# bytewax/bytewax

Hardware: AMD Instinct MI355X
Metric: events/sec (whole node), tumbling-window wordcount (higher is better)
Workload: dtype int64; 1 GPU; model=tumbling-window wordcount (keyed count, 60s windows), events_per_batch_per_gpu=64000000, vocab=1000000, parallelism=key-hash all-to-allv dp1, engine=dataflow (run_main: source -> keyed_window_agg -> sink), radix=True, radix_v2=False, latency_method=poll-gap under load, closed_window_rows=317000000

## Files before the change

### bytewax_amd/_native/stream_kernels.hip

```cpp

#include <hip/hip_runtime.h>
#include <torch/extension.h>
#include <pybind11/stl.h>
#include <ATen/hip/HIPContext.h>

#include <chrono>
#include <type_traits>
#include <cstdlib>
#include <cstdint>
#include <cstring>
#include <vector>

#define WAVE 64
#define EMPTY_SLOT 0xFFFFFFFFFFFFFFFFULL

#define HIP_CHECK(expr)                                               \
  do {                                                                \
    hipError_t _e = (expr);                                           \
    TORCH_CHECK(_e == hipSuccess, "HIP error: ", hipGetErrorString(_e)); \
  } while (0)

static inline int n_blocks(int64_t n, int block) {
  int64_t b = (n + block - 1) / block;
  if (b > 2048) b = 2048;
// ... 349 lines not shown
      int rp = atomicAdd(&gres[b], 1);
      if (rp < res_cap) {
        ev_res[(int64_t)b * res_cap + rp] = stage[b][q];
      } else {
        atomicOr(error_flag, 1);
      }
    }
  }
  for (int off = WAVE / 2; off > 0; off >>= 1) {
    int64_t other = __shfl_down((long long)local_max, off);
    if (other > local_max) local_max = other;
  }
  if ((threadIdx.x & (WAVE - 1)) == 0 && local_max > 0) {
    atomicMax(max_ts, (unsigned long long)local_max);
  }
}

#define V2_CACHE 4096

__global__ __launch_bounds__(256) void k_agg_cached(
    const uint64_t* __restrict__ ev,
    const uint64_t* __restrict__ ev_res,
    const int* __restrict__ gcur,
    const int* __restrict__ gres,
    int64_t cap_c,
    int64_t res_cap,
    int slices,
    uint64_t* __restrict__ tkeys,
    unsigned long long* __restrict__ tvals,
    uint64_t mask,
    int region_bits,
    int* __restrict__ error_flag) {
  __shared__ uint64_t ckeys[V2_CACHE];
  __shared__ unsigned long long cvals[V2_CACHE];
  for (int s = threadIdx.x; s < V2_CACHE; s += blockDim.x) {
    ckeys[s] = EMPTY_SLOT;
    cvals[s] = 0;
  }
  __syncthreads();
  int cb = blockIdx.x % V2_COARSE;
  int slice = blockIdx.x / V2_COARSE;

  auto agg_one = [&](uint64_t packed) {
    uint64_t h64 = mix64(packed);
    int lh = (int)((h64 >> 20) & (V2_CACHE - 1));
    for (int p = 0; p < 2; ++p) {
      uint64_t cur = ckeys[lh];
      if (cur == packed) {
        atomicAdd(&cvals[lh], 1ULL);
        return;
      }
      if (cur == EMPTY_SLOT) {
        uint64_t prev = atomicCAS(
            (unsigned long long*)&ckeys[lh], EMPTY_SLOT, packed);
        if (prev == EMPTY_SLOT || prev == packed) {
          atomicAdd(&cvals[lh], 1ULL);
          return;
        }
      }
      lh = (lh + 1) & (V2_CACHE - 1);
    }
    if (!hash_add(tkeys, tvals, mask, region_bits, packed, 1ULL)) {
      atomicOr(error_flag, 1);
    }
  };

  int c = gcur[cb];
  if (c > cap_c) c = (int)cap_c;
  for (int j = slice * (int)blockDim.x + threadIdx.x; j < c;
       j += slices * (int)blockDim.x) {
    agg_one(ev[(int64_t)cb * cap_c + j]);
  }
  int cr = gres[cb];
  if (cr > res_cap) cr = (int)res_cap;
  for (int j = slice * (int)blockDim.x + threadIdx.x; j < cr;
       j += slices * (int)blockDim.x) {
    agg_one(ev_res[(int64_t)cb * res_cap + j]);
  }
  __syncthreads();
  for (int s = threadIdx.x; s < V2_CACHE; s += blockDim.x) {
    if (ckeys[s] != EMPTY_SLOT) {
      if (!hash_add(tkeys, tvals, mask, region_bits, ckeys[s], cvals[s])) {
        atomicOr(error_flag, 1);
      }
    }
  }
}

__device__ __forceinline__ int64_t win_lo_of(
    int64_t t, int64_t align_ms, int64_t len_ms, int64_t off_ms) {
  int64_t num = t - align_ms - len_ms;
  int64_t fl = num >= 0 ? num / off_ms : -((-num + off_ms - 1) / off_ms);
  return fl + 1;
}

__device__ __forceinline__ int64_t win_of(
    int64_t t, int64_t align_ms, int64_t len_ms, uint64_t m2,
    uint64_t maxfast) {
  int64_t x = t - align_ms;
  if (m2 != 0 && (uint64_t)x < maxfast) {
    return (int64_t)__umul64hi((uint64_t)x, m2);
  }
  return x / len_ms;
}

static inline void magic_div_u64(
    int64_t d, uint64_t* m2, uint64_t* maxfast) {
  *m2 = 0;
  *maxfast = 0;
  if (d <= 1) return;
  if ((d & (d - 1)) == 0) {
    int s = 0;
    while ((int64_t(1) << s) < d) ++s;
    *m2 = (uint64_t)1 << (64 - s);
    *maxfast = ~(uint64_t)0;
    return;
  }
  const unsigned p = 60;
  unsigned __int128 one = 1;
  uint64_t M = (uint64_t)(((one << p) + (uint64_t)d - 1) / (uint64_t)d);
  uint64_t e = (uint64_t)((unsigned __int128)M * (uint64_t)d - (one << p));
  *m2 = M << 4;
  *maxfast = e ? (uint64_t)((one << p) / e) : ~(uint64_t)0;
}

struct Win32 {
  uint32_t dlo;
  uint32_t dspan;
  uint32_t c;
  uint32_t wlo;
  uint32_t qoff;
  uint32_t dm;
  int sh1, sh2;
};

__device__ __forceinline__ uint32_t win32_div(uint32_t y, const Win32& w) {
  uint32_t t = __umulhi(w.dm, y);
  return (t + ((y - t) >> w.sh1)) >> w.sh2;
}

#define ENTRY_SLOT_BITS 13
#define ENTRY_SLOT_MASK 0x1FFFull
#define ENTRY_DELTA_MASK 0x7FFFFu
#define ENTRY_DELTA_LIMIT 0x7FFFFu
#define ENTRY_W_CLASSIC INT64_MIN

__device__ __forceinline__ uint32_t entry_delta(uint64_t entry) {
  return ((uint32_t)entry >> ENTRY_SLOT_BITS) & ENTRY_DELTA_MASK;
}

__device__ __forceinline__ uint64_t entry_classic(
    uint64_t entry, uint32_t wlo) {
  return ((uint64_t)(wlo + entry_delta(entry)) << 32) | (entry >> 32);
}

template <int MODE, typename TS = int64_t, bool LATE = false>
__global__ void k_radix_scatter_fixed(
    const int32_t* __restrict__ keys,
    const TS* __restrict__ ts,
    const int64_t* __restrict__ vals,
    int64_t n,
    int64_t align_ms,
    int64_t len_ms,
    int64_t off_ms,
    int64_t ts_base,
    uint64_t mask,
    int region_bits,
    int64_t cap,
    int* __restrict__ gcursors,
    uint64_t* __restrict__ ev_packed,
    int64_t* __restrict__ ev_vals,
    int* __restrict__ ov_cursor,
    uint64_t* __restrict__ ov_packed,
    int64_t* __restrict__ ov_vals,
    int64_t ov_cap,
    unsigned long long* __restrict__ max_ts,
    int* __restrict__ error_flag,
    uint64_t win_m2,
    uint64_t win_maxfast,
    int64_t late_cutoff,
    int32_t* __restrict__ late_keys,
    int64_t* __restrict__ late_ts,
    int64_t* __restrict__ late_vals,
    int* __restrict__ late_n,
    int64_t late_cap) {
  static_assert(!(LATE && MODE == AGG_TS), "no late tracking for AGG_TS");
  extern __shared__ int lmem[];
  __shared__ int s_late[LATE ? 2 : 1];
  int nb = (int)(((mask + 1) >> region_bits));
  int* lhist = lmem;
  int* lbase = lmem + nb;
  for (int b = threadIdx.x; b < nb; b += blockDim.x) lhist[b] = 0;
  if constexpr (LATE) {
    if (threadIdx.x == 0) s_late[0] = 0;
  }
  __syncthreads();
  int64_t start = blockIdx.x * (int64_t)blockDim.x + threadIdx.x;
  int64_t stride = gridDim.x * (int64_t)blockDim.x;
  int64_t local_max = 0;
  for (int64_t i = start; i < n; i += stride) {
    int64_t t = (int64_t)ts[i] + ts_base;
    if constexpr (LATE) {
      bool is_late = t < late_cutoff;
      wave_reserve(is_late, &s_late[0]);
      if (is_late) continue;
    }
    if (t > local_max) local_max = t;
    uint64_t packed;
    int nwin = 1;
    if (MODE == AGG_TS) {
      packed = (uint64_t)(uint32_t)keys[i];
    } else {
      int64_t win = win_of(t, align_ms, off_ms, win_m2, win_maxfast);
      packed = ((uint64_t)(uint32_t)(int32_t)win << 32) | (uint32_t)keys[i];
      if (off_ms < len_ms) {
        nwin = (int)(win - win_lo_of(t, align_ms, len_ms, off_ms)) + 1;
      }
    }
    for (int w = 0; w < nwin; ++w) {
      atomicAdd(&lhist[(int)region_of(mix64(packed), mask, region_bits)], 1);
      packed -= (uint64_t)1 << 32;
    }
  }
  __syncthreads();
  for (int b = threadIdx.x; b < nb; b += blockDim.x) {
    lbase[b] = lhist[b] > 0 ? atomicAdd(&gcursors[b], lhist[b]) : 0;
    lhist[b] = 0;
  }
  if constexpr (LATE) {
    if (threadIdx.x == 0) {
      s_late[1] = s_late[0] > 0 ? atomicAdd(late_n, s_late[0]) : 0;
      s_late[0] = 0;
    }
  }
  __syncthreads();
  for (int64_t i = start; i < n; i += stride) {
    int64_t t = (int64_t)ts[i] + ts_base;
    if constexpr (LATE) {
      bool is_late = t < late_cutoff;
      int lpos = wave_reserve(is_late, &s_late[0]);
      if (is_late) {
        late_store<MODE == AGG_SUM>(
            (int64_t)s_late[1] + lpos, keys[i], t,
            MODE == AGG_SUM ? vals[i] : 0, late_keys, late_ts, late_vals,
            late_cap, error_flag);
        continue;
      }
    }
    uint64_t packed;
    int nwin = 1;
    if (MODE == AGG_TS) {
      packed = (uint64_t)(uint32_t)keys[i];
    } else {
      int64_t win = win_of(t, align_ms, off_ms, win_m2, win_maxfast);
      packed = ((uint64_t)(uint32_t)(int32_t)win << 32) | (uint32_t)keys[i];
      if (off_ms < len_ms) {
        nwin = (int)(win - win_lo_of(t, align_ms, len_ms, off_ms)) + 1;
      }
    }
    int64_t v = (MODE == AGG_SUM) ? vals[i] : (MODE == AGG_TS ? t : 0);
    for (int w = 0; w < nwin; ++w) {
      int b = (int)region_of(mix64(packed), mask, region_bits);
      int64_t in_bucket = lbase[b] + atomicAdd(&lhist[b], 1);
      if (in_bucket < cap) {
        int64_t pos = (int64_t)b * cap + in_bucket;
        ev_packed[pos] = packed;
        if (MODE != AGG_COUNT) ev_vals[pos] = v;
      } else {
        int opos = atomicAdd(ov_cursor, 1);
        if (opos < ov_cap) {
          ov_packed[opos] = packed;
          if (MODE != AGG_COUNT) ov_vals[opos] = v;
        } else {
          atomicOr(error_flag, 1);
        }
      }
      packed -= (uint64_t)1 << 32;
    }
  }
  for (int off = WAVE / 2; off > 0; off >>= 1) {
    int64_t other = __shfl_down((long long)local_max, off);
    if (other > local_max) local_max = other;
  }
  if ((threadIdx.x & (WAVE - 1)) == 0 && local_max > 0) {
    atomicMax(max_ts, (unsigned long long)local_max);
  }
}

template <int MODE, typename TS = int64_t>
__global__ void k_radix_scatter_direct(
    const int32_t* __restrict__ keys,
    const TS* __restrict__ ts,
    const int64_t* __restrict__ vals,
    int64_t n,
    int64_t align_ms,
    int64_t len_ms,
    int64_t off_ms,
    int64_t ts_base,
    uint64_t mask,
    int region_bits,
    int64_t cap,
    int* __restrict__ gcursors,
    uint64_t* __restrict__ ev_packed,
    int64_t* __restrict__ ev_vals,
    int* __restrict__ ov_cursor,
    uint64_t* __restrict__ ov_packed,
// ... 324 lines not shown
      int64_t i = t0 + u * BLK + tid;
      if (i > n - 1) i = n - 1;
      rk[u] = keys[i];
      rt[u] = ts[i];
    }
  };
  const int64_t stride = (int64_t)gridDim.x * T;
  int64_t local_max = 0;
  int64_t t0 = (int64_t)blockIdx.x * T;
  const bool seen = t0 + tid < n;
  if (t0 < n) {
    load_tile(t0);
    if (HASHED) local_max = (int64_t)rt[0];
  }
  for (; t0 < n; t0 += stride) {
    uint64_t pk[U];
    int sr[U];
    if (!HASHED) {
#pragma unroll
      for (int u = 0; u < U; ++u) {
        int64_t i = t0 + u * BLK + tid;
        int64_t t = (int64_t)rt[u] + ts_base;
        int64_t win = win_of(t, align_ms, len_ms, win_m2, win_maxfast);
        uint64_t packed =
            ((uint64_t)(uint32_t)(int32_t)win << 32) | (uint32_t)rk[u];
        pk[u] = packed;
        int b = (int)region_of(mix64(packed), mask, seg_bits);
        sr[u] = -1;
        if (i < n) {
          if (t > local_max) local_max = t;
          sr[u] = (atomicAdd(&lhist[b], 1) << 13) | b;
        }
      }
    } else {
      int64_t left64 = n - t0 - tid;
      const int left = left64 > T ? T : (left64 < 0 ? 0 : (int)left64);
      int32_t dmax = (int32_t)local_max;
      uint32_t rare = 0;
#pragma unroll
      for (int u = 0; u < U; ++u) {
        const bool in = u * BLK < left;
        const uint32_t d = (uint32_t)rt[u];
        const uint32_t q = win32_div(d + w32.c, w32);
        const uint64_t packed =
            ((uint64_t)(w32.wlo + q) << 32) | (uint32_t)rk[u];
        const uint64_t h64 = mix64(packed);
        const uint32_t delta = q - w32.qoff;
        const bool fits =
            d - w32.dlo < w32.dspan && delta < ENTRY_DELTA_LIMIT;
        pk[u] = ((uint64_t)(uint32_t)rk[u] << 32) |
                (uint64_t)(delta << ENTRY_SLOT_BITS) |
                ((h64 >> 32) & ENTRY_SLOT_MASK);
        if (in && !fits) rare |= 1u << u;
        if (in && (int32_t)d > dmax) dmax = (int32_t)d;
        const bool ok = in && fits;
        int b = (int)region_of(h64, mask, seg_bits);
        int rank = atomicAdd(&lhist[b], ok ? 1 : 0);
        sr[u] = ok ? ((rank << 13) | b) : -1;
      }
      local_max = dmax;
      while (rare != 0) {
        int u = __ffs(rare) - 1;
        rare &= rare - 1;
        int64_t i = t0 + u * BLK + tid;
        int64_t win = win_of((int64_t)ts[i] + ts_base, align_ms, len_ms,
                             win_m2, win_maxfast);
        spill(((uint64_t)(uint32_t)(int32_t)win << 32) | (uint32_t)keys[i]);
      }
    }
    if (t0 + stride < n) load_tile(t0 + stride);
    __syncthreads();
    int rc = 0, grant = 0, gb = 0;
    if (tid < nseg) {
      rc = res_cnt[tid];
      int tot = rc + lhist[tid];
      grant = tot & ~(SC_GRAN - 1);
      if (grant > 0) gb = atomicAdd(&gcursors[tid], grant);
      res_cnt[tid] = tot - grant;
      lhist[tid] = 0;
    }
    int incl = grant;
    for (int o = 1; o < WAVE; o <<= 1) {
      int v = __shfl_up(incl, o);
      if (lane >= o) incl += v;
    }
    if (lane == WAVE - 1) s_wtot[wave] = incl;
    __syncthreads();
    int total = 0, woff = 0;
    for (int w = 0; w < NW; ++w) {
      int v = s_wtot[w];
      if (w < wave) woff += v;
      total += v;
    }
    if (tid < nseg) {
      int off = woff + incl - grant;
      lpack[tid] = off | (rc << 14) | (grant << 17);
      if (grant > 0) {
#pragma unroll
        for (int j = 0; j < SC_GRAN - 1; ++j)
          stage[off + j] = res[(size_t)tid * SC_GRAN + j];
        for (int j = 0; j < grant; j += SC_GRAN) {
          int64_t gp = (int64_t)gb + j;
          gdst[(off + j) / SC_GRAN] =
              gp < cap ? (uint32_t)(((int64_t)tid * cap + gp) / SC_GRAN)
                       : GD_SPILL;
        }
      }
    }
    __syncthreads();
    for (int u = 0; u < U; ++u) {
      if (sr[u] < 0) continue;
      int b = sr[u] & ((1 << 13) - 1);
      int w = lpack[b];
      int vpos = ((w >> 14) & 7) + (sr[u] >> 13);
      int g = w >> 17;
      if (vpos < g) stage[(w & ((1 << 14) - 1)) + vpos] = pk[u];
      else res[(size_t)b * SC_GRAN + (vpos - g)] = pk[u];
    }
    __syncthreads();
    for (int p = tid; p < total / 2; p += BLK) {
      ulonglong2 v = *(const ulonglong2*)(stage + 2 * p);
      uint32_t d = gdst[p / 4];
      if (d != GD_SPILL) {
        *(ulonglong2*)(ev_packed + (int64_t)d * SC_GRAN + 2 * (p & 3)) = v;
      } else {
        if (v.x != EMPTY_SLOT) spill(classic_of(v.x));
        if (v.y != EMPTY_SLOT) spill(classic_of(v.y));
      }
    }
  }
  __syncthreads();
  if (tid < nseg) {
    int rc = res_cnt[tid];
    if (rc > 0) {
      int gb = atomicAdd(&gcursors[tid], SC_GRAN);
      for (int j = 0; j < SC_GRAN; ++j) {
        uint64_t p = j < rc ? res[(size_t)tid * SC_GRAN + j] : EMPTY_SLOT;
        int64_t gp = (int64_t)gb + j;
        if (gp < cap) ev_packed[(int64_t)tid * cap + gp] = p;
        else if (p != EMPTY_SLOT) spill(classic_of(p));
      }
    }
  }
  if (HASHED) local_max = seen ? local_max + ts_base : 0;
  for (int off = WAVE / 2; off > 0; off >>= 1) {
    int64_t other = __shfl_down((long long)local_max, off);
    if (other > local_max) local_max = other;
  }
  if ((threadIdx.x & (WAVE - 1)) == 0 && local_max > 0) {
    atomicMax(max_ts, (unsigned long long)local_max);
  }
}

template <int MODE>
__global__ void k_overflow_agg(
    const uint64_t* __restrict__ ov_packed,
    const int64_t* __restrict__ ov_vals,
    const int* __restrict__ ov_cursor,
    int64_t ov_cap,
    uint64_t* __restrict__ tkeys,
    unsigned long long* __restrict__ tvals,
    uint64_t mask,
    int region_bits,
    int* __restrict__ error_flag) {
  int64_t n = *ov_cursor;
  if (n > ov_cap) n = ov_cap;
  int64_t i = blockIdx.x * (int64_t)blockDim.x + threadIdx.x;
  int64_t stride = gridDim.x * (int64_t)blockDim.x;
  for (; i < n; i += stride) {
    unsigned long long inc =
        (MODE == AGG_SUM) ? (unsigned long long)ov_vals[i] : 1ULL;
    if (!hash_add(tkeys, tvals, mask, region_bits, ov_packed[i], inc)) {
      atomicOr(error_flag, 1);
    }
  }
}

typedef unsigned long long agg_u64x2 __attribute__((ext_vector_type(2)));

template <int MODE>
__global__ __launch_bounds__(1024) void k_radix_agg(
    const uint64_t* __restrict__ ev_packed,
    const int64_t* __restrict__ ev_vals,
    const int* __restrict__ counts,
    int64_t cap,
    uint64_t* __restrict__ tkeys,
    unsigned long long* __restrict__ tvals,
    uint64_t mask,
    int region_bits,
    int lds_bits,
    int* __restrict__ error_flag) {
  extern __shared__ char smem[];
  int region = 1 << lds_bits;
  uint64_t* lkeys = (uint64_t*)smem;
  unsigned long long* lvals =
      (unsigned long long*)(smem + (size_t)region * sizeof(uint64_t));
  for (int s = threadIdx.x; s < region; s += blockDim.x) {
    lkeys[s] = EMPTY_SLOT;
    lvals[s] = 0;
  }
  __syncthreads();
  int b = blockIdx.x;
  int cnt = counts[b];
  if (cnt > (int)cap) cnt = (int)cap;
  const uint64_t* seg = ev_packed + (int64_t)b * cap;
  const int64_t* segv =
      (MODE == AGG_SUM) ? ev_vals + (int64_t)b * cap : nullptr;

  auto add = [&](uint64_t packed, unsigned long long inc) {
    if (packed == EMPTY_SLOT) return;
    uint64_t h64 = mix64(packed);
    int lh = (int)((h64 >> 32) & (region - 1));
    bool done = false;
    for (int p = 0; p < region; ++p) {
      uint64_t cur = lkeys[lh];
      if (cur == packed) {
        atomicAdd(&lvals[lh], inc);
        done = true;
        break;
      }
      if (cur == EMPTY_SLOT) {
        uint64_t prev = atomicCAS(
            (unsigned long long*)&lkeys[lh], EMPTY_SLOT, packed);
        if (prev == EMPTY_SLOT || prev == packed) {
          atomicAdd(&lvals[lh], inc);
          done = true;
          break;
        }
      }
      lh = (lh + 1) & (region - 1);
    }
    if (!done) {
      if (!hash_add(tkeys, tvals, mask, region_bits, packed, inc)) {
        atomicOr(error_flag, 1);
      }
    }
  };

  const int head = (cnt > 0 && ((uintptr_t)seg & 15) != 0) ? 1 : 0;
  const int nvec = (cnt - head) >> 1;
  const int tail = head + 2 * nvec;
  if (threadIdx.x == 0 && head) {
    add(seg[0], MODE == AGG_SUM ? (unsigned long long)segv[0] : 1ULL);
  }
  if (threadIdx.x == blockDim.x - 1 && tail < cnt) {
    add(seg[tail],
        MODE == AGG_SUM ? (unsigned long long)segv[tail] : 1ULL);
  }

  constexpr int R = (MODE == AGG_SUM) ? 2 : 4;
  const agg_u64x2* vseg = (const agg_u64x2*)(seg + head);
  const int64_t* vval = (MODE == AGG_SUM) ? segv + head : nullptr;
  const int T = (int)blockDim.x;
  const int chunk = R * T;
  agg_u64x2 cur_p[R], nxt_p[R];
  unsigned long long cur_v[R][2], nxt_v[R][2];
  auto fetch = [&](agg_u64x2 (&bp)[R], unsigned long long (&bv)[R][2],
                   int base) {
#pragma unroll
    for (int r = 0; r < R; ++r) {
      int v = base + r * T + (int)threadIdx.x;
      if (v < nvec) {
        bp[r] = vseg[v];
        if (MODE == AGG_SUM) {
          bv[r][0] = (unsigned long long)vval[2 * v];
          bv[r][1] = (unsigned long long)vval[2 * v + 1];
        }
      } else {
        bp[r] = agg_u64x2{EMPTY_SLOT, EMPTY_SLOT};
        if (MODE == AGG_SUM) bv[r][0] = bv[r][1] = 0;
      }
    }
  };
  if (nvec > 0) fetch(cur_p, cur_v, 0);
  for (int base = 0; base < nvec; base += chunk) {
    if (base + chunk < nvec) fetch(nxt_p, nxt_v, base + chunk);
#pragma unroll
    for (int r = 0; r < R; ++r) {
      add(cur_p[r].x, MODE == AGG_SUM ? cur_v[r][0] : 1ULL);
      add(cur_p[r].y, MODE == AGG_SUM ? cur_v[r][1] : 1ULL);
    }
#pragma unroll
    for (int r = 0; r < R; ++r) {
      cur_p[r] = nxt_p[r];
      if (MODE == AGG_SUM) {
        cur_v[r][0] = nxt_v[r][0];
        cur_v[r][1] = nxt_v[r][1];
      }
    }
  }
  __syncthreads();
  for (int s = threadIdx.x; s < region; s += blockDim.x) {
    if (lkeys[s] != EMPTY_SLOT) {
      if (!hash_add(tkeys, tvals, mask, region_bits, lkeys[s], lvals[s])) {
        atomicOr(error_flag, 1);
      }
    }
  }
}

#define AGG_DELTA_MAX 14u
#define AGG_DELTA_MID 7u

template <int BLK, int R, bool HASHED = false>
__global__ __launch_bounds__(BLK, BLK == 1024 ? 8 : 4) void k_radix_agg_count(
    const uint64_t* __restrict__ ev_packed,
    const int* __restrict__ counts,
    int64_t cap,
    uint64_t* __restrict__ tkeys,
    unsigned long long* __restrict__ tvals,
    uint64_t mask,
    int region_bits,
    int lds_bits,
    int* __restrict__ error_flag,
    uint32_t wlo) {
  extern __shared__ char smem[];
  unsigned long long* cells = (unsigned long long*)smem;
  const int region = 1 << lds_bits;
  const uint32_t lmask = (uint32_t)region - 1;
  const int b = blockIdx.x;
  int cnt = counts[b];
  if (cnt > (int)cap) cnt = (int)cap;
  if (cnt <= 0) return;
  for (int s = threadIdx.x; s < region / 2; s += BLK) {
    ((agg_u64x2*)cells)[s] = agg_u64x2{EMPTY_SLOT, EMPTY_SLOT};
  }
  const uint64_t* seg = ev_packed + (int64_t)b * cap;
  auto win_part = [&](uint64_t packed) {
    return HASHED ? entry_delta(packed) : (uint32_t)(packed >> 32);
  };
  auto key_part = [&](uint64_t packed) {
    return HASHED ? (uint32_t)(packed >> 32) : (uint32_t)packed;
  };
  const uint32_t wbase = win_part(seg[0]) - AGG_DELTA_MID;
  __syncthreads();

  auto escape = [&](uint64_t packed) {
    if (HASHED) packed = entry_classic(packed, wlo);
    if (!hash_add(tkeys, tvals, mask, region_bits, packed, 1ULL)) {
      atomicOr(error_flag, 1);
    }
  };
  auto slot_of = [&](uint64_t packed) {
    if (HASHED) return (uint32_t)packed & lmask;
    return (uint32_t)(mix64(packed) >> 32) & lmask;
  };
  auto tag_of = [&](uint64_t packed) {
    return ((unsigned long long)key_part(packed) << 4) |
           (unsigned long long)(win_part(packed) - wbase);
  };
  auto drain = [&](uint32_t pend, auto entry, auto start, auto skipped) {
    uint64_t packed = 0;
    unsigned long long tag = 0;
    uint32_t lh = 0;
    int left = 0;
    while (left != 0 || pend != 0) {
      if (left == 0) {
        int e = __ffs(pend) - 1;
        pend &= pend - 1;
        packed = entry(e);
        if (win_part(packed) - wbase > AGG_DELTA_MAX) {
          escape(packed);
          continue;
        }
        tag = tag_of(packed);
        lh = start(e);
        left = region - (skipped(e) ? 1 : 0);
      }
      unsigned long long cur = cells[lh];
      if (cur == EMPTY_SLOT) {
        cur = atomicCAS(&cells[lh], EMPTY_SLOT, tag << 28);
        if (cur == EMPTY_SLOT) cur = tag << 28;
      }
      if ((cur >> 28) == tag) {
        atomicAdd((unsigned int*)&cells[lh], 1u);
        left = 0;
      } else {
        lh = (lh + 1) & lmask;
        if (--left == 0) escape(packed);
      }
    }
  };
  auto add_one = [&](uint64_t packed) {
    if (packed == EMPTY_SLOT) return;
    drain(
        1u, [&](int) { return packed; },
        [&](int) { return slot_of(packed); }, [&](int) { return false; });
  };

  const int head = ((uintptr_t)seg & 15) != 0 ? 1 : 0;
  const int nvec = (cnt - head) >> 1;
  const int tail = head + 2 * nvec;
  if (threadIdx.x == 0 && head) add_one(seg[0]);
  if (threadIdx.x == BLK - 1 && tail < cnt) add_one(seg[tail]);

  const agg_u64x2* vseg = (const agg_u64x2*)(seg + head);
  constexpr int chunk = R * BLK;
  constexpr int E = 2 * R;
  agg_u64x2 cur_p[R], nxt_p[R];
  auto fetch = [&](agg_u64x2 (&bp)[R], int base) {
#pragma unroll
    for (int r = 0; r < R; ++r) {
      int v = base + r * BLK + (int)threadIdx.x;
      if (v < nvec) bp[r] = vseg[v];
      else bp[r] = agg_u64x2{EMPTY_SLOT, EMPTY_SLOT};
    }
  };
  fetch(cur_p, 0);
  for (int base = 0; base < nvec; base += chunk) {
    if (base + chunk < nvec) fetch(nxt_p, base + chunk);
    uint32_t slot[E];
    unsigned long long first[E];
#pragma unroll
    for (int e = 0; e < E; ++e) {
      uint64_t packed = (e & 1) ? cur_p[e >> 1].y : cur_p[e >> 1].x;
      slot[e] = slot_of(packed);
      first[e] = cells[slot[e]];
    }
    uint32_t pend = 0, moved = 0;
#pragma unroll
    for (int e = 0; e < E; ++e) {
      uint64_t packed = (e & 1) ? cur_p[e >> 1].y : cur_p[e >> 1].x;
      if (packed == EMPTY_SLOT) continue;
      bool in_range = win_part(packed) - wbase <= AGG_DELTA_MAX;
      if (in_range && (first[e] >> 28) == tag_of(packed)) {
        atomicAdd((unsigned int*)&cells[slot[e]], 1u);
      } else {
        pend |= 1u << e;
        if (first[e] != EMPTY_SLOT) {
          slot[e] = (slot[e] + 1) & lmask;
          moved |= 1u << e;
        }
      }
    }
    if (pend != 0) {
      drain(
          pend,
          [&](int e) {
            uint64_t v = 0;
#pragma unroll
            for (int j = 0; j < E; ++j) {
              if (j == e) v = (j & 1) ? cur_p[j >> 1].y : cur_p[j >> 1].x;
            }
            return v;
          },
          [&](int e) {
            uint32_t v = 0;
#pragma unroll
            for (int j = 0; j < E; ++j) {
              if (j == e) v = slot[j];
            }
            return v;
          },
          [&](int e) { return ((moved >> e) & 1u) != 0; });
    }
#pragma unroll
    for (int r = 0; r < R; ++r) cur_p[r] = nxt_p[r];
  }
  __syncthreads();

  for (int s = threadIdx.x; s < region; s += BLK) {
    unsigned long long c = cells[s];
    if (c != EMPTY_SLOT) {
      uint32_t win = wbase + ((uint32_t)c >> 28) + (HASHED ? wlo : 0u);
      uint64_t packed = ((uint64_t)win << 32) | (c >> 32);
      if (!hash_add(tkeys, tvals, mask, region_bits, packed,
                    c & 0x0FFFFFFFULL)) {
        atomicOr(error_flag, 1);
      }
    }
  }
}

__global__ void k_overflow_agg_stats(
    const uint64_t* __restrict__ ov_packed,
    const int64_t* __restrict__ ov_vals,
    const int* __restrict__ ov_cursor,
    int64_t ov_cap,
    uint64_t* __restrict__ tkeys,
    long long* __restrict__ tcnt,
    long long* __restrict__ tsum,
    long long* __restrict__ tmin,
    long long* __restrict__ tmax,
    uint64_t mask,
    int* __restrict__ error_flag) {
  int64_t n = *ov_cursor;
  if (n > ov_cap) n = ov_cap;
  int64_t i = blockIdx.x * (int64_t)blockDim.x + threadIdx.x;
  int64_t stride = gridDim.x * (int64_t)blockDim.x;
  for (; i < n; i += stride) {
    uint64_t slot = find_slot(tkeys, mask, ov_packed[i]);
    if (slot == ~0ULL) {
      atomicOr(error_flag, 1);
      continue;
    }
    long long v = ov_vals[i];
    atomicAdd((unsigned long long*)&tcnt[slot], 1ULL);
    atomicAdd((unsigned long long*)&tsum[slot], (unsigned long long)v);
    atomicMin(&tmin[slot], v);
    atomicMax(&tmax[slot], v);
  }
}

__global__ __launch_bounds__(1024) void k_radix_agg_stats(
    const uint64_t* __restrict__ ev_packed,
    const int64_t* __restrict__ ev_vals,
    const int* __restrict__ offsets,
    const int* __restrict__ counts,
    uint64_t* __restrict__ tkeys,
    long long* __restrict__ tcnt,
    long long* __restrict__ tsum,
    long long* __restrict__ tmin,
    long long* __restrict__ tmax,
    int64_t clamp_cap,
    uint64_t mask,
    int region_bits,
    int lds_bits,
    int* __restrict__ error_flag) {
  extern __shared__ char smem[];
  int region = 1 << lds_bits;
  uint64_t* lkeys = (uint64_t*)smem;
  long long* lcnt = (long long*)(smem + (size_t)region * 8);
  long long* lsum = (long long*)(smem + (size_t)region * 16);
  long long* lmin = (long long*)(smem + (size_t)region * 24);
  long long* lmax = (long long*)(smem + (size_t)region * 32);
  const long long LLMAX = 0x7FFFFFFFFFFFFFFFLL;
  for (int s = threadIdx.x; s < region; s += blockDim.x) {
    lkeys[s] = EMPTY_SLOT;
    lcnt[s] = 0;
    lsum[s] = 0;
    lmin[s] = LLMAX;
    lmax[s] = -LLMAX - 1;
  }
  __syncthreads();
  int b = blockIdx.x;
  int cnt = counts[b];
  if (clamp_cap > 0 && cnt > (int)clamp_cap) cnt = (int)clamp_cap;
  int start = offsets[b];
  for (int j = threadIdx.x; j < cnt; j += blockDim.x) {
    uint64_t packed = ev_packed[start + j];
    if (packed == EMPTY_SLOT) continue;
    long long v = ev_vals[start + j];
    uint64_t h64 = mix64(packed);
    int lh = (int)((h64 >> 32) & (region - 1));
    int slot = -1;
    for (int p = 0; p < region; ++p) {
      uint64_t cur = lkeys[lh];
      if (cur == packed) {
        slot = lh;
        break;
      }
      if (cur == EMPTY_SLOT) {
        uint64_t prev = atomicCAS(
            (unsigned long long*)&lkeys[lh], EMPTY_SLOT, packed);
        if (prev == EMPTY_SLOT || prev == packed) {
          slot = lh;
          break;
        }
      }
      lh = (lh + 1) & (region - 1);
    }
    if (slot >= 0) {
      atomicAdd((unsigned long long*)&lcnt[slot], 1ULL);
      atomicAdd((unsigned long long*)&lsum[slot], (unsigned long long)v);
      atomicMin(&lmin[slot], v);
      atomicMax(&lmax[slot], v);
    } else {
      uint64_t gslot = find_slot(tkeys, mask, packed);
      if (gslot == ~0ULL) {
        atomicOr(error_flag, 1);
      } else {
        atomicAdd((unsigned long long*)&tcnt[gslot], 1ULL);
        atomicAdd((unsigned long long*)&tsum[gslot], (unsigned long long)v);
        atomicMin(&tmin[gslot], v);
        atomicMax(&tmax[gslot], v);
      }
    }
  }
  __syncthreads();
  for (int s = threadIdx.x; s < region; s += blockDim.x) {
    if (lkeys[s] != EMPTY_SLOT) {
      uint64_t gslot = find_slot(tkeys, mask, lkeys[s]);
      if (gslot == ~0ULL) {
        atomicOr(error_flag, 1);
        continue;
      }
      atomicAdd((unsigned long long*)&tcnt[gslot],
                (unsigned long long)lcnt[s]);
      atomicAdd((unsigned long long*)&tsum[gslot],
                (unsigned long long)lsum[s]);
      atomicMin(&tmin[gslot], lmin[s]);
      atomicMax(&tmax[gslot], lmax[s]);
    }
  }
}

__global__ void k_close_extract(
    const uint64_t* __restrict__ tkeys,
    const unsigned long long* __restrict__ tvals,
    int64_t nslots,
    int64_t win_lo,
    int64_t win_hi,
    int32_t* __restrict__ out_keys,
    int32_t* __restrict__ out_wins,
    int64_t* __restrict__ out_vals,
    int* __restrict__ out_n,
    int64_t cap) {
  int64_t i = blockIdx.x * (int64_t)blockDim.x + threadIdx.x;
  int64_t stride = gridDim.x * (int64_t)blockDim.x;
  for (; i < nslots; i += stride) {
    uint64_t k = tkeys[i];
    bool take = false;
    int32_t win = 0;
    if (k != EMPTY_SLOT) {
      win = (int32_t)(uint32_t)(k >> 32);
      take = (int64_t)win >= win_lo && (int64_t)win < win_hi;
    }
    unsigned long long ball = __ballot(take);
    int lane = threadIdx.x & (WAVE - 1);
    if (ball != 0) {
// ... 1433 lines not shown
  return LateSink{late_cutoff, late_keys.data_ptr<int32_t>(),
                  late_ts.data_ptr<int64_t>(), vp,
                  late_n.data_ptr<int32_t>(), cap};
}

static void window_agg_insert_impl(
    torch::Tensor keys,
    torch::Tensor ts,
    c10::optional<torch::Tensor> vals,
    torch::Tensor tkeys,
    torch::Tensor tvals,
    torch::Tensor max_ts,
    torch::Tensor error_flag,
    int64_t align_ms,
    int64_t len_ms,
    int64_t mode,
    bool dedup,
    int64_t ts_base,
    int64_t region_bits,
    int64_t off_ms,
    const LateSink* late) {
  TORCH_CHECK(late == nullptr || !dedup,
              "late tracking is incompatible with the dedup path");
  if (off_ms <= 0) off_ms = len_ms;
  TORCH_CHECK(off_ms <= len_ms, "window offset must be <= length");
  TORCH_CHECK(off_ms == len_ms || !dedup,
              "sliding windows are incompatible with the dedup path");
  check_dev(keys, torch::kInt32, "keys");
  bool ts32 = ts.scalar_type() == torch::kInt32;
  if (!ts32) check_dev(ts, torch::kInt64, "ts");
  check_dev(tkeys, torch::kInt64, "tkeys");
  check_dev(tvals, torch::kInt64, "tvals");
  check_dev(max_ts, torch::kInt64, "max_ts");
  check_dev(error_flag, torch::kInt32, "error_flag");
  int64_t n = keys.numel();
  TORCH_CHECK(ts.numel() == n, "ts/keys length mismatch");
  int64_t nslots = tkeys.numel();
  TORCH_CHECK((nslots & (nslots - 1)) == 0, "table size must be 2^k");
  TORCH_CHECK(len_ms > 0, "window length must be positive");
  const int64_t* vptr = nullptr;
  if (mode == AGG_SUM) {
    TORCH_CHECK(vals.has_value(), "sum mode requires vals");
    check_dev(*vals, torch::kInt64, "vals");
    TORCH_CHECK(vals->numel() == n, "vals/keys length mismatch");
    vptr = vals->data_ptr<int64_t>();
  }
  if (n == 0) return;
  auto stream = at::hip::getCurrentHIPStream();
  dim3 block(256);
  dim3 grid(n_blocks(n, 256));
  auto launch = [&](auto kern, auto tsptr) {
    hipLaunchKernelGGL(
        kern, grid, block, 0, stream,
        keys.data_ptr<int32_t>(), tsptr, vptr, n,
        (uint64_t*)tkeys.data_ptr<int64_t>(),
        (unsigned long long*)tvals.data_ptr<int64_t>(),
        (uint64_t)(nslots - 1), align_ms, len_ms, off_ms, ts_base,
        (int)region_bits,
        (unsigned long long*)max_ts.data_ptr<int64_t>(),
        error_flag.data_ptr<int32_t>(), (const int64_t*)nullptr,
        late ? late->cutoff : (int64_t)0, late ? late->keys : nullptr,
        late ? late->ts : nullptr, late ? late->vals : nullptr,
        late ? late->n : nullptr, late ? late->cap : (int64_t)0);
  };
  auto dispatch = [&](auto tsptr) {
    using TSV = std::remove_const_t<std::remove_pointer_t<decltype(tsptr)>>;
    if (late != nullptr && mode == AGG_COUNT)
      launch((k_window_agg_insert<AGG_COUNT, false, TSV, true>), tsptr);
    else if (late != nullptr)
      launch((k_window_agg_insert<AGG_SUM, false, TSV, true>), tsptr);
    else if (mode == AGG_COUNT && !dedup)
      launch(k_window_agg_insert<AGG_COUNT, false, TSV>, tsptr);
    else if (mode == AGG_COUNT && dedup)
      launch(k_window_agg_insert<AGG_COUNT, true, TSV>, tsptr);
    else if (mode == AGG_SUM && !dedup)
      launch(k_window_agg_insert<AGG_SUM, false, TSV>, tsptr);
    else
      launch(k_window_agg_insert<AGG_SUM, true, TSV>, tsptr);
  };
  if (ts32) dispatch(ts.data_ptr<int32_t>());
  else dispatch(ts.data_ptr<int64_t>());
}

void window_agg_insert(
    torch::Tensor keys,
    torch::Tensor ts,
    c10::optional<torch::Tensor> vals,
    torch::Tensor tkeys,
    torch::Tensor tvals,
    torch::Tensor max_ts,
    torch::Tensor error_flag,
    int64_t align_ms,
    int64_t len_ms,
    int64_t mode,
    bool dedup,
    int64_t ts_base,
    int64_t region_bits,
    int64_t off_ms) {
  window_agg_insert_impl(keys, ts, vals, tkeys, tvals, max_ts, error_flag,
                         align_ms, len_ms, mode, dedup, ts_base, region_bits,
                         off_ms, nullptr);
}

void window_agg_insert_late(
    torch::Tensor keys,
    torch::Tensor ts,
    c10::optional<torch::Tensor> vals,
    torch::Tensor tkeys,
    torch::Tensor tvals,
    torch::Tensor max_ts,
    torch::Tensor error_flag,
    int64_t align_ms,
    int64_t len_ms,
    int64_t mode,
    int64_t ts_base,
    int64_t region_bits,
    int64_t off_ms,
    int64_t late_cutoff,
    torch::Tensor late_keys,
    torch::Tensor late_ts,
    c10::optional<torch::Tensor> late_vals,
    torch::Tensor late_n) {
  LateSink sink = make_late_sink(late_cutoff, late_keys, late_ts, late_vals,
                                 late_n, mode == AGG_SUM);
  window_agg_insert_impl(keys, ts, vals, tkeys, tvals, max_ts, error_flag,
                         align_ms, len_ms, mode, false, ts_base, region_bits,
                         off_ms, &sink);
}

static unsigned device_cu_count() {
  static int cus = 0;
  if (cus == 0) {
    int dev = 0, v = 0;
    if (hipGetDevice(&dev) == hipSuccess &&
        hipDeviceGetAttribute(&v, hipDeviceAttributeMultiprocessorCount,
                              dev) == hipSuccess &&
        v > 0)
      cus = v;
    else
      cus = 256;
  }
  return (unsigned)cus;
}

static bool agg_wide_env() {
  const char* s = std::getenv("BYTEWAX_AGG");
  return s != nullptr && s[0] == 'w';
}

static bool entries_classic_env() {
  const char* s = std::getenv("BYTEWAX_ENTRIES");
  return s != nullptr && s[0] == 'c';
}

static bool staged2_shape(int64_t nseg, int* threads, int* u, size_t* lds) {
  int env_u = 0, env_threads = 0;
  if (const char* e = std::getenv("BYTEWAX_SCATTER_U")) env_u = atoi(e);
  if (const char* e = std::getenv("BYTEWAX_SCATTER_THREADS"))
    env_threads = atoi(e);
  *threads = env_threads == 1024 ? 1024 : 512;
  *u = *threads == 512 && env_u != 8 ? 16 : 8;
  *lds = staged2_lds_bytes(nseg, (int64_t)*threads * *u);
  return nseg <= *threads && *lds <= 160 * 1024;
}

static bool count_staged2_ok(int64_t xf, const void* evp, int64_t nseg) {
  int threads, u;
  size_t lds;
  return xf == 1 && scatter_staged2_env() && (((uintptr_t)evp) & 15) == 0 &&
         staged2_shape(nseg, &threads, &u, &lds);
}

static bool count_agg_compact(int64_t cap, int seg_bits) {
  return !agg_wide_env() && cap < ((int64_t)1 << 28) && seg_bits >= 8 &&
         seg_bits <= 13;
}

struct CountEntries {
  bool hashed = false;
  int64_t W = 0;
  uint32_t qoff = 0;
  uint32_t dm = 0;
  int sh1 = 0, sh2 = 0;
  int64_t agg_w() const {
    return hashed ? W + (int64_t)qoff : ENTRY_W_CLASSIC;
  }
};

static CountEntries plan_count_entries(
    bool staged_count, int64_t xf, const void* evp, int64_t nseg,
    int64_t cap, int seg_bits, bool ts_i32, int64_t align_ms,
    int64_t len_ms, int64_t first_base) {
  CountEntries ce;
  if (!staged_count || !ts_i32 || entries_classic_env() ||
      !count_staged2_ok(xf, evp, nseg) || !count_agg_compact(cap, seg_bits))
    return ce;
  if (len_ms < 1 || len_ms >= ((int64_t)1 << 31)) return ce;
  int threads, u;
  size_t lds;
  staged2_shape(nseg, &threads, &u, &lds);
  if (threads != 512 || u != 16) return ce;
  __int128 num = (__int128)first_base - align_ms - ((__int128)1 << 31);
  __int128 w = num / len_ms;
  if (num % len_ms < 0) w -= 1;
  if (w < -((__int128)1 << 62) || w > ((__int128)1 << 62)) return ce;
  ce.hashed = true;
  ce.W = (int64_t)w;
  int l = 0;
  while (((int64_t)1 << l) < len_ms) ++l;
  ce.dm = (uint32_t)((((unsigned __int128)1 << 32) *
                      (uint64_t)(((int64_t)1 << l) - len_ms)) /
                     (uint64_t)len_ms) + 1u;
  ce.sh1 = l < 1 ? l : 1;
  ce.sh2 = l > 1 ? l - 1 : 0;
  int64_t q0 = (int64_t)((num - w * len_ms + ((__int128)1 << 31)) / len_ms);
  ce.qoff = q0 > (1 << 18) ? (uint32_t)(q0 - (1 << 18)) : 0u;
  return ce;
}

static Win32 make_win32(
    const CountEntries& ce, int64_t ts_base, int64_t align_ms,
    int64_t len_ms) {
  Win32 w{};
  __int128 c = (__int128)ts_base - align_ms - (__int128)ce.W * len_ms;
  __int128 lo = -((__int128)1 << 31), hi = ((__int128)1 << 31) - 1;
  if (-c > lo) lo = -c;
  if ((__int128)align_ms - ts_base > lo) lo = (__int128)align_ms - ts_base;
  __int128 top = ((__int128)1 << 32) - 1 - c;
  if (top < hi) hi = top;
  if (hi >= lo) {
    __int128 span = hi - lo + 1;
    if (span > 0xFFFFFFFFll) span = 0xFFFFFFFFll;
    w.dlo = (uint32_t)(int32_t)(int64_t)lo;
    w.dspan = (uint32_t)(uint64_t)span;
  }
  w.c = (uint32_t)(uint64_t)(c & 0xFFFFFFFFll);
  w.wlo = (uint32_t)(uint64_t)ce.W;
  w.qoff = ce.qoff;
  w.dm = ce.dm;
  w.sh1 = ce.sh1;
  w.sh2 = ce.sh2;
  return w;
}

template <typename TSV>
static void launch_count_staged(
    hipStream_t stream, const int32_t* keys, const TSV* ts, int64_t n,
    int64_t xf, int64_t align_ms, int64_t len_ms, int64_t off_ms,
    int64_t ts_base, uint64_t mask, int seg_bits, int64_t nseg, int64_t cap,
    int* gcur, uint64_t* evp, int* ovc, uint64_t* ovp, int64_t ov_cap,
    unsigned long long* max_ts, int* err, uint64_t win_m2,
    uint64_t win_maxfast, bool overlapped, const CountEntries& ce) {
  int env_u = 0, env_threads = 0, env_blocks = 0;
  if (const char* e = std::getenv("BYTEWAX_SCATTER_U")) env_u = atoi(e);
  if (const char* e = std::getenv("BYTEWAX_SCATTER_THREADS"))
    env_threads = atoi(e);
  if (const char* e = std::getenv("BYTEWAX_SCATTER_BLOCKS")) {
    int v = atoi(e);
    if (v > 0) env_blocks = v;
  }
  auto go = [&](auto kern, int threads, int u, unsigned cap_gs, size_t lds,
                auto... extra) {
    int64_t tile = (int64_t)threads * u;
    int64_t gs = (n * xf + tile - 1) / tile;
    if (env_blocks > 0) cap_gs = (unsigned)env_blocks;
    if (gs > (int64_t)cap_gs) gs = cap_gs;
    if (gs < 1) gs = 1;
    hipLaunchKernelGGL(
        kern, dim3((unsigned)gs), dim3((unsigned)threads), lds, stream, keys,
        ts, (const int64_t*)nullptr, n, align_ms, len_ms, off_ms, ts_base,
        mask, seg_bits, cap, gcur, evp, (int64_t*)nullptr, ovc, ovp,
        (int64_t*)nullptr, ov_cap, max_ts, err, win_m2, win_maxfast,
        extra...);
    HIP_CHECK(hipGetLastError());
  };
  TORCH_CHECK(!ce.hashed || count_staged2_ok(xf, evp, nseg),
              "hashed entries planned for a scatter that is not staged2");
  if (count_staged2_ok(xf, evp, nseg)) {
    const unsigned cus = device_cu_count() * (overlapped ? 2u : 1u);
    int threads, u;
    size_t lds;
    staged2_shape(nseg, &threads, &u, &lds);
    Win32 w32{};
    if constexpr (sizeof(TSV) == 4) {
      if (ce.hashed) {
        w32 = make_win32(ce, ts_base, align_ms, len_ms);
        go((k_radix_scatter_staged2<TSV, 16, 512, true>), 512, 16, cus, lds,
           w32);
        return;
      }
    }
    TORCH_CHECK(!ce.hashed, "hashed entries need int32 timestamp deltas");
    if (threads == 1024)
      go((k_radix_scatter_staged2<TSV, 8, 1024>), 1024, 8, cus, lds, w32);
    else if (u == 16)
      go((k_radix_scatter_staged2<TSV, 16, 512>), 512, 16, cus, lds, w32);
    else
      go((k_radix_scatter_staged2<TSV, 8, 512>), 512, 8, cus, lds, w32);
    return;
  }
  size_t lds = (size_t)nseg * SC_GRAN * 8 + 4 * (size_t)nseg * sizeof(int);
  int threads = 512;
  if (env_threads == 256 || env_threads == 1024) threads = env_threads;
  if (threads == 512)
    go((k_radix_scatter_staged<AGG_COUNT, TSV, 16, 512>), 512, 16, 1024u,
       lds, NO_LATE_ARGS);
  else if (threads == 1024)
    go((k_radix_scatter_staged<AGG_COUNT, TSV, 16, 1024>), 1024, 16, 1024u,
       lds, NO_LATE_ARGS);
  else if (env_u == 8)
    go((k_radix_scatter_staged<AGG_COUNT, TSV, 8>), 256, 8, 1024u, lds,
       NO_LATE_ARGS);
  else if (env_u == 32)
    go((k_radix_scatter_staged<AGG_COUNT, TSV, 32>), 256, 32, 1024u, lds,
       NO_LATE_ARGS);
  else
    go((k_radix_scatter_staged<AGG_COUNT, TSV, 16>), 256, 16, 1024u, lds,
       NO_LATE_ARGS);
}

static void launch_count_agg(
    hipStream_t stream, const uint64_t* evp, const int* gcur, int64_t cap,
    uint64_t* tkeys, unsigned long long* tvals, uint64_t mask,
    int region_bits, int seg_bits, int64_t nseg, int* err,
    int64_t entry_w) {
  const bool hashed = entry_w != ENTRY_W_CLASSIC;
  const uint32_t wlo = hashed ? (uint32_t)(uint64_t)entry_w : 0u;
  if (count_agg_compact(cap, seg_bits)) {
    auto go = [&](auto kern, int threads) {
      hipLaunchKernelGGL(
          kern, dim3((unsigned)nseg), dim3((unsigned)threads),
          (size_t)8 << seg_bits, stream, evp, gcur, cap, tkeys, tvals, mask,
          region_bits, seg_bits, err, wlo);
      HIP_CHECK(hipGetLastError());
    };
    if (seg_bits >= 12) {
      if (hashed) go((k_radix_agg_count<1024, 2, true>), 1024);
      else go((k_radix_agg_count<1024, 2>), 1024);
    } else {
      if (hashed) go((k_radix_agg_count<256, 2, true>), 256);
      else go((k_radix_agg_count<256, 2>), 256);
    }
    return;
  }
  TORCH_CHECK(!hashed, "hashed scatter entries need the compact aggregation");
  hipLaunchKernelGGL(
      k_radix_agg<AGG_COUNT>, dim3((unsigned)nseg),
      dim3(seg_bits >= 12 ? 1024u : 256u), (size_t)16 << seg_bits, stream,
      evp, (const int64_t*)nullptr, gcur, cap, tkeys, tvals, mask,
      region_bits, seg_bits, err);
  HIP_CHECK(hipGetLastError());
}

static dim3 overflow_agg_grid() { return dim3(device_cu_count()); }

static void radix_window_insert_impl(
    torch::Tensor keys,
    torch::Tensor ts,
    c10::optional<torch::Tensor> vals,
    torch::Tensor tkeys,
    torch::Tensor tvals,
    torch::Tensor max_ts,
    torch::Tensor error_flag,
    torch::Tensor gcursors,
    torch::Tensor ev_packed,
    torch::Tensor ev_vals,
    torch::Tensor ov_cursor,
    torch::Tensor ov_packed,
    torch::Tensor ov_vals,
    int64_t align_ms,
    int64_t len_ms,
    int64_t mode,
    int64_t ts_base,
    int64_t region_bits,
    int64_t off_ms,
    std::vector<int64_t> seg_counts,
    std::vector<int64_t> seg_bases,
    const LateSink* late) {
  if (off_ms <= 0) off_ms = len_ms;
  TORCH_CHECK(off_ms <= len_ms, "window offset must be <= length");
  check_dev(keys, torch::kInt32, "keys");
  bool seg32 = !seg_counts.empty();
  bool ts32 = ts.scalar_type() == torch::kInt32;
  if (seg32) {
    TORCH_CHECK(seg_counts.size() == seg_bases.size(),
                "seg_counts/seg_bases length mismatch");
    check_dev(ts, torch::kInt32, "ts32");
  } else if (!ts32) {
    check_dev(ts, torch::kInt64, "ts");
  }
  int64_t n = keys.numel();
  int64_t nslots = tkeys.numel();
  TORCH_CHECK((nslots & (nslots - 1)) == 0, "table size must be 2^k");
  TORCH_CHECK(region_bits > 0, "radix path requires region_bits > 0");
  TORCH_CHECK(region_bits <= 12, "region_bits > 12 exceeds the LDS "
              "budget of the aggregation kernel (16 B/slot)");
  int64_t nb = nslots >> region_bits;
  TORCH_CHECK(nb >= 1 && nb <= 8192, "region count out of range");
  TORCH_CHECK(gcursors.numel() >= nb, "gcursors too small");
  const int64_t* vptr = nullptr;
  if (mode == AGG_SUM) {
    TORCH_CHECK(vals.has_value(), "sum mode requires vals");
    vptr = vals->data_ptr<int64_t>();
  }
  if (n == 0) return;
  auto stream = at::hip::getCurrentHIPStream();
  uint64_t mask = (uint64_t)(nslots - 1);
  dim3 block(256);
  dim3 grid(n_blocks(n, 256));

  ScatterKind kind = scatter_kind_env();
  int64_t xf = off_ms < len_ms ? (len_ms + off_ms - 1) / off_ms : 1;
  TORCH_CHECK(xf <= 64, "sliding expansion > 64x; use a larger offset");
  if (kind == SCAT_DIRECT && xf > 1) kind = SCAT_FIXED;
  if (late != nullptr && kind == SCAT_DIRECT) kind = SCAT_FIXED;
  int coarse = scatter_coarse_bits(kind);
  int seg_bits = (int)region_bits + coarse;
  int64_t nseg = nslots >> seg_bits;
  size_t staged_lds = (size_t)nseg * SC_GRAN * 8 *
                          (mode == AGG_SUM ? 2 : 1) +
                      4 * (size_t)nseg * sizeof(int);
  const size_t late_lds = late != nullptr ? 2 * sizeof(int) : 0;
  while (kind == SCAT_STAGED &&
         (nseg < 1 || staged_lds + late_lds > 160 * 1024 ||
          seg_bits > 13)) {
    if (coarse > 0 && seg_bits > 13) {
      coarse -= 1;
    } else {
      kind = SCAT_FIXED;
      coarse = 0;
    }
    seg_bits = (int)region_bits + coarse;
    nseg = nslots >> seg_bits;
    staged_lds = (size_t)nseg * SC_GRAN * 8 * (mode == AGG_SUM ? 2 : 1) +
                 4 * (size_t)nseg * sizeof(int);
  }
  if (seg_bits > 13) {
    coarse = 0;
    seg_bits = (int)region_bits;
    nseg = nb;
  }
  int64_t cap = ev_packed.numel() / nseg;
  if (kind == SCAT_STAGED) {
    cap &= ~(int64_t)(SC_GRAN - 1);
    if (cap < SC_GRAN) {
      kind = SCAT_FIXED;
      coarse = 0;
      seg_bits = (int)region_bits;
      nseg = nb;
      cap = ev_packed.numel() / nseg;
    }
  }
  TORCH_CHECK(cap * nseg >= 2 * n * xf || cap >= n * xf,
              "scatter buffers too small (need ~2x batch x expansion)");
  if (mode == AGG_SUM) {
    TORCH_CHECK(ev_vals.numel() >= nseg * cap, "ev_vals too small");
  }
  gcursors.narrow(0, 0, nseg).zero_();
  ov_cursor.zero_();
  size_t hist_lds = (size_t)nseg * sizeof(int);

  int env_blocks = 0;
  if (const char* sb = std::getenv("BYTEWAX_SCATTER_BLOCKS")) {
    int v = atoi(sb);
    if (v > 0) env_blocks = v;
  }

  struct Seg {
    int64_t off, n, base;
  };
  std::vector<Seg> segs;
  if (seg32) {
    int64_t off = 0;
    for (size_t i = 0; i < seg_counts.size(); ++i) {
      if (seg_counts[i] > 0) segs.push_back({off, seg_counts[i], seg_bases[i]});
      off += seg_counts[i];
    }
    TORCH_CHECK(off == n, "segment counts must sum to batch length");
  } else {
    segs.push_back({0, n, ts_base});
  }

  uint64_t win_m2, win_maxfast;
  magic_div_u64(off_ms, &win_m2, &win_maxfast);
  const CountEntries ce = plan_count_entries(
      kind == SCAT_STAGED && mode == AGG_COUNT && late == nullptr, xf,
      ev_packed.data_ptr<int64_t>(), nseg, cap, seg_bits, seg32 || ts32,
      align_ms, len_ms, segs[0].base);
  unsigned scat_threads = 256;
  auto scat = [&](auto kern, auto tsptr, const Seg& sg, unsigned gx,
                  size_t lds, auto... extra) {
    hipLaunchKernelGGL(
        kern, dim3(gx), dim3(scat_threads), lds, stream,
        keys.data_ptr<int32_t>() + sg.off, tsptr + sg.off,
        vptr != nullptr ? vptr + sg.off : nullptr, sg.n, align_ms, len_ms,
        off_ms, sg.base, mask, seg_bits, cap, gcursors.data_ptr<int32_t>(),
        (uint64_t*)ev_packed.data_ptr<int64_t>(),
        mode == AGG_SUM ? ev_vals.data_ptr<int64_t>() : nullptr,
        ov_cursor.data_ptr<int32_t>(),
        (uint64_t*)ov_packed.data_ptr<int64_t>(),
        mode == AGG_SUM ? ov_vals.data_ptr<int64_t>() : nullptr,
        ov_packed.numel(),
        (unsigned long long*)max_ts.data_ptr<int64_t>(),
        error_flag.data_ptr<int32_t>(), win_m2, win_maxfast, extra...);
    HIP_CHECK(hipGetLastError());
  };
  auto scat_late = [&](auto tsptr, const Seg& sg) {
    using TSV = std::remove_const_t<std::remove_pointer_t<decltype(tsptr)>>;
    if (kind == SCAT_STAGED) {
      int sthreads = mode == AGG_COUNT ? 512 : 256;
      scat_threads = (unsigned)sthreads;
      unsigned gs =
          (unsigned)((sg.n * xf + sthreads * 16 - 1) / (sthreads * 16));
      if (gs > 1024u) gs = 1024u;
      if (gs < 1) gs = 1;
      if (mode == AGG_COUNT)
        scat((k_radix_scatter_staged<AGG_COUNT, TSV, 16, 512, true>), tsptr,
             sg, gs, staged_lds, late->cutoff, late->keys, late->ts,
             late->vals, late->n, late->cap);
      else
        scat((k_radix_scatter_staged<AGG_SUM, TSV, 16, 256, true>), tsptr,
             sg, gs, staged_lds, late->cutoff, late->keys, late->ts,
             late->vals, late->n, late->cap);
    } else {
      scat_threads = 256;
      unsigned gx = (unsigned)n_blocks(sg.n, 256);
      if (mode == AGG_COUNT)
        scat((k_radix_scatter_fixed<AGG_COUNT, TSV, true>), tsptr, sg, gx,
             2 * hist_lds, late->cutoff, late->keys, late->ts, late->vals,
             late->n, late->cap);
      else
        scat((k_radix_scatter_fixed<AGG_SUM, TSV, true>), tsptr, sg, gx,
             2 * hist_lds, late->cutoff, late->keys, late->ts, late->vals,
             late->n, late->cap);
    }
  };
  auto scat_any = [&](auto tsptr, const Seg& sg) {
    using TSV = std::remove_const_t<std::remove_pointer_t<decltype(tsptr)>>;
    if (late != nullptr) {
      scat_late(tsptr, sg);
      return;
    }
    unsigned gx = (unsigned)n_blocks(sg.n, 256);
    if (env_blocks > 0 && (unsigned)env_blocks < gx) gx = (unsigned)env_blocks;
    if (kind == SCAT_STAGED) {
      if (mode == AGG_COUNT) {
        launch_count_staged<TSV>(
            stream, keys.data_ptr<int32_t>() + sg.off, tsptr + sg.off, sg.n,
            xf, align_ms, len_ms, off_ms, sg.base, mask, seg_bits, nseg, cap,
            gcursors.data_ptr<int32_t>(),
            (uint64_t*)ev_packed.data_ptr<int64_t>(),
            ov_cursor.data_ptr<int32_t>(),
            (uint64_t*)ov_packed.data_ptr<int64_t>(), ov_packed.numel(),
            (unsigned long long*)max_ts.data_ptr<int64_t>(),
            error_flag.data_ptr<int32_t>(), win_m2, win_maxfast,
            false, ce);
      } else {
        unsigned cap_gs = env_blocks > 0 ? (unsigned)env_blocks : 1024u;
        unsigned gs = (unsigned)((sg.n * xf + 256 * 16 - 1) / (256 * 16));
        if (gs > cap_gs) gs = cap_gs;
        if (gs < 1) gs = 1;
        scat_threads = 256;
        scat(k_radix_scatter_staged<AGG_SUM, TSV>, tsptr, sg, gs,
             staged_lds, NO_LATE_ARGS);
      }
    } else if (kind == SCAT_DIRECT) {
      scat_threads = 256;
      if (mode == AGG_COUNT)
        scat(k_radix_scatter_direct<AGG_COUNT, TSV>, tsptr, sg, gx, 0);
      else
        scat(k_radix_scatter_direct<AGG_SUM, TSV>, tsptr, sg, gx, 0);
    } else {
      scat_threads = 256;
      if (mode == AGG_COUNT)
        scat(k_radix_scatter_fixed<AGG_COUNT, TSV>, tsptr, sg, gx,
             2 * hist_lds, NO_LATE_ARGS);
      else
        scat(k_radix_scatter_fixed<AGG_SUM, TSV>, tsptr, sg, gx,
             2 * hist_lds, NO_LATE_ARGS);
    }
  };
  for (const Seg& sg : segs) {
    if (seg32 || ts32) scat_any(ts.data_ptr<int32_t>(), sg);
    else scat_any(ts.data_ptr<int64_t>(), sg);
  }

  size_t agg_lds = (size_t)16 << seg_bits;
  dim3 agg_block(seg_bits >= 12 ? 1024 : 256);
  auto agg = [&](auto kern) {
    hipLaunchKernelGGL(
        kern, dim3((unsigned)nseg), agg_block, agg_lds, stream,
        (const uint64_t*)ev_packed.data_ptr<int64_t>(),
        mode == AGG_SUM ? ev_vals.data_ptr<int64_t>() : nullptr,
        gcursors.data_ptr<int32_t>(), cap,
        (uint64_t*)tkeys.data_ptr<int64_t>(),
        (unsigned long long*)tvals.data_ptr<int64_t>(), mask,
        (int)region_bits, seg_bits, error_flag.data_ptr<int32_t>());
  };
  if (mode == AGG_COUNT) {
    launch_count_agg(
        stream, (const uint64_t*)ev_packed.data_ptr<int64_t>(),
        gcursors.data_ptr<int32_t>(), cap,
        (uint64_t*)tkeys.data_ptr<int64_t>(),
        (unsigned long long*)tvals.data_ptr<int64_t>(), mask,
        (int)region_bits, seg_bits, nseg, error_flag.data_ptr<int32_t>(),
        ce.agg_w());
  } else {
    agg(k_radix_agg<AGG_SUM>);
  }

  auto ov = [&](auto kern) {
    hipLaunchKernelGGL(
        kern, overflow_agg_grid(), dim3(256), 0, stream,
        (const uint64_t*)ov_packed.data_ptr<int64_t>(),
        mode == AGG_SUM ? ov_vals.data_ptr<int64_t>() : nullptr,
        ov_cursor.data_ptr<int32_t>(), ov_packed.numel(),
        (uint64_t*)tkeys.data_ptr<int64_t>(),
        (unsigned long long*)tvals.data_ptr<int64_t>(), mask,
        (int)region_bits, error_flag.data_ptr<int32_t>());
  };
  if (mode == AGG_COUNT) ov(k_overflow_agg<AGG_COUNT>);
  else ov(k_overflow_agg<AGG_SUM>);
}

void radix_window_insert(
    torch::Tensor keys,
    torch::Tensor ts,
    c10::optional<torch::Tensor> vals,
    torch::Tensor tkeys,
    torch::Tensor tvals,
    torch::Tensor max_ts,
    torch::Tensor error_flag,
    torch::Tensor gcursors,
    torch::Tensor ev_packed,
    torch::Tensor ev_vals,
    torch::Tensor ov_cursor,
    torch::Tensor ov_packed,
    torch::Tensor ov_vals,
    int64_t align_ms,
    int64_t len_ms,
    int64_t mode,
    int64_t ts_base,
    int64_t region_bits,
    int64_t off_ms = 0,
    std::vector<int64_t> seg_counts = {},
    std::vector<int64_t> seg_bases = {}) {
  radix_window_insert_impl(
      keys, ts, vals, tkeys, tvals, max_ts, error_flag, gcursors, ev_packed,
      ev_vals, ov_cursor, ov_packed, ov_vals, align_ms, len_ms, mode, ts_base,
      region_bits, off_ms, std::move(seg_counts), std::move(seg_bases),
      nullptr);
}

void radix_window_insert_late(
    torch::Tensor keys,
    torch::Tensor ts,
    c10::optional<torch::Tensor> vals,
    torch::Tensor tkeys,
    torch::Tensor tvals,
    torch::Tensor max_ts,
    torch::Tensor error_flag,
    torch::Tensor gcursors,
    torch::Tensor ev_packed,
    torch::Tensor ev_vals,
    torch::Tensor ov_cursor,
    torch::Tensor ov_packed,
    torch::Tensor ov_vals,
    int64_t align_ms,
    int64_t len_ms,
    int64_t mode,
    int64_t ts_base,
    int64_t region_bits,
    int64_t off_ms,
    int64_t late_cutoff,
    torch::Tensor late_keys,
    torch::Tensor late_ts,
    c10::optional<torch::Tensor> late_vals,
    torch::Tensor late_n) {
  LateSink sink = make_late_sink(late_cutoff, late_keys, late_ts, late_vals,
                                 late_n, mode == AGG_SUM);
  radix_window_insert_impl(
      keys, ts, vals, tkeys, tvals, max_ts, error_flag, gcursors, ev_packed,
      ev_vals, ov_cursor, ov_packed, ov_vals, align_ms, len_ms, mode, ts_base,
      region_bits, off_ms, {}, {}, &sink);
}

int64_t radix_scatter_only(
    torch::Tensor keys,
    torch::Tensor ts,
    c10::optional<torch::Tensor> vals,
    torch::Tensor max_ts,
    torch::Tensor error_flag,
    torch::Tensor gcursors,
    torch::Tensor ev_packed,
    torch::Tensor ev_vals,
    torch::Tensor ov_cursor,
    torch::Tensor ov_packed,
    torch::Tensor ov_vals,
    int64_t nslots,
    int64_t align_ms,
    int64_t len_ms,
    int64_t mode,
    int64_t ts_base,
    int64_t region_bits,
    int64_t off_ms,
    std::vector<int64_t> seg_counts,
    std::vector<int64_t> seg_bases) {
  if (off_ms <= 0) off_ms = len_ms;
  TORCH_CHECK(off_ms <= len_ms, "window offset must be <= length");
  check_dev(keys, torch::kInt32, "keys");
  bool seg32 = !seg_counts.empty();
  bool ts32 = ts.scalar_type() == torch::kInt32;
  if (seg32) {
    TORCH_CHECK(seg_counts.size() == seg_bases.size(),
                "seg_counts/seg_bases length mismatch");
    check_dev(ts, torch::kInt32, "ts32");
  } else if (!ts32) {
    check_dev(ts, torch::kInt64, "ts");
  }
  int64_t n = keys.numel();
  TORCH_CHECK((nslots & (nslots - 1)) == 0, "table size must be 2^k");
  int64_t nb = nslots >> region_bits;
  const int64_t* vptr = nullptr;
  if (mode == AGG_SUM) {
    TORCH_CHECK(vals.has_value(), "sum mode requires vals");
    vptr = vals->data_ptr<int64_t>();
  }
  auto stream = at::hip::getCurrentHIPStream();
  uint64_t mask = (uint64_t)(nslots - 1);
  dim3 block(256);
  uint64_t win_m2, win_maxfast;
  magic_div_u64(off_ms <= 0 ? len_ms : off_ms, &win_m2, &win_maxfast);

  ScatterKind kind = scatter_kind_env();
  int64_t xf = off_ms < len_ms ? (len_ms + off_ms - 1) / off_ms : 1;
  TORCH_CHECK(xf <= 64, "sliding expansion > 64x; use a larger offset");
  if (kind == SCAT_DIRECT && xf > 1) kind = SCAT_FIXED;
  int coarse = scatter_coarse_bits(kind);
  int seg_bits = (int)region_bits + coarse;
  int64_t nseg = nslots >> seg_bits;
  size_t staged_lds = (size_t)nseg * SC_GRAN * 8 *
                          (mode == AGG_SUM ? 2 : 1) +
                      4 * (size_t)nseg * sizeof(int);
  while (kind == SCAT_STAGED &&
         (nseg < 1 || staged_lds > 160 * 1024 || seg_bits > 13)) {
    if (coarse > 0 && seg_bits > 13) {
      coarse -= 1;
    } else {
      kind = SCAT_FIXED;
      coarse = 0;
    }
    seg_bits = (int)region_bits + coarse;
    nseg = nslots >> seg_bits;
    staged_lds = (size_t)nseg * SC_GRAN * 8 * (mode == AGG_SUM ? 2 : 1) +
                 4 * (size_t)nseg * sizeof(int);
  }
  if (seg_bits > 13) {
    coarse = 0;
    seg_bits = (int)region_bits;
    nseg = nb;
  }
  int64_t cap = ev_packed.numel() / nseg;
  if (kind == SCAT_STAGED) {
    cap &= ~(int64_t)(SC_GRAN - 1);
    if (cap < SC_GRAN) {
      kind = SCAT_FIXED;
      coarse = 0;
      seg_bits = (int)region_bits;
      nseg = nb;
      cap = ev_packed.numel() / nseg;
    }
  }
  TORCH_CHECK(cap * nseg >= 2 * n * xf || cap >= n * xf,
              "scatter buffers too small");
  size_t hist_lds = (size_t)nseg * sizeof(int);
  HIP_CHECK(hipMemsetAsync(
      gcursors.data_ptr<int32_t>(), 0, (size_t)nseg * sizeof(int), stream));
  HIP_CHECK(hipMemsetAsync(
      ov_cursor.data_ptr<int32_t>(), 0, sizeof(int), stream));
  if (n == 0) return ENTRY_W_CLASSIC;

  struct Seg {
    int64_t off, n, base;
  };
  std::vector<Seg> segs;
  if (seg32) {
    int64_t off = 0;
    for (size_t i = 0; i < seg_counts.size(); ++i) {
      if (seg_counts[i] > 0) segs.push_back({off, seg_counts[i], seg_bases[i]});
      off += seg_counts[i];
    }
  } else {
    segs.push_back({0, n, ts_base});
  }
  if (segs.empty()) return ENTRY_W_CLASSIC;
  const CountEntries ce = plan_count_entries(
      kind == SCAT_STAGED && mode == AGG_COUNT, xf,
      ev_packed.data_ptr<int64_t>(), nseg, cap, seg_bits, seg32 || ts32,
      align_ms, len_ms, segs[0].base);
  unsigned scat_threads = 256;
  auto scat = [&](auto kern, auto tsptr, const Seg& sg, unsigned gx,
                  size_t lds, auto... extra) {
    hipLaunchKernelGGL(
        kern, dim3(gx), dim3(scat_threads), lds,
        stream, keys.data_ptr<int32_t>() + sg.off, tsptr + sg.off,
        vptr != nullptr ? vptr + sg.off : nullptr, sg.n, align_ms, len_ms,
        off_ms, sg.base, mask, seg_bits, cap, gcursors.data_ptr<int32_t>(),
        (uint64_t*)ev_packed.data_ptr<int64_t>(),
        mode == AGG_SUM ? ev_vals.data_ptr<int64_t>() : nullptr,
        ov_cursor.data_ptr<int32_t>(),
        (uint64_t*)ov_packed.data_ptr<int64_t>(),
        mode == AGG_SUM ? ov_vals.data_ptr<int64_t>() : nullptr,
        ov_packed.numel(),
        (unsigned long long*)max_ts.data_ptr<int64_t>(),
        error_flag.data_ptr<int32_t>(), win_m2, win_maxfast, extra...);
  };
  auto scat_any = [&](auto tsptr, const Seg& sg) {
    using TSV = std::remove_const_t<std::remove_pointer_t<decltype(tsptr)>>;
    if (kind == SCAT_STAGED) {
      if (mode == AGG_COUNT) {
        launch_count_staged<TSV>(
            stream, keys.data_ptr<int32_t>() + sg.off, tsptr + sg.off, sg.n,
            xf, align_ms, len_ms, off_ms, sg.base, mask, seg_bits, nseg, cap,
            gcursors.data_ptr<int32_t>(),
            (uint64_t*)ev_packed.data_ptr<int64_t>(),
            ov_cursor.data_ptr<int32_t>(),
            (uint64_t*)ov_packed.data_ptr<int64_t>(), ov_packed.numel(),
            (unsigned long long*)max_ts.data_ptr<int64_t>(),
            error_flag.data_ptr<int32_t>(), win_m2, win_maxfast,
            true, ce);
      } else {
        unsigned gs = (unsigned)((sg.n + 4095) / 4096);
        if (gs > 1024) gs = 1024;
        if (gs < 1) gs = 1;
        scat(k_radix_scatter_staged<AGG_SUM, TSV>, tsptr, sg, gs,
             staged_lds, NO_LATE_ARGS);
      }
    } else if (kind == SCAT_DIRECT) {
      unsigned gx = (unsigned)n_blocks(sg.n, 256);
      if (mode == AGG_COUNT)
        scat(k_radix_scatter_direct<AGG_COUNT, TSV>, tsptr, sg, gx, 0);
      else
        scat(k_radix_scatter_direct<AGG_SUM, TSV>, tsptr, sg, gx, 0);
    } else {
      unsigned gx = (unsigned)n_blocks(sg.n, 256);
      if (mode == AGG_COUNT)
        scat(k_radix_scatter_fixed<AGG_COUNT, TSV>, tsptr, sg, gx,
             2 * hist_lds, NO_LATE_ARGS);
      else
        scat(k_radix_scatter_fixed<AGG_SUM, TSV>, tsptr, sg, gx,
             2 * hist_lds, NO_LATE_ARGS);
    }
  };
  for (const Seg& sg : segs) {
    if (seg32 || ts32) scat_any(ts.data_ptr<int32_t>(), sg);
    else scat_any(ts.data_ptr<int64_t>(), sg);
  }
  return ce.agg_w();
}

void radix_agg_only(
    torch::Tensor tkeys,
    torch::Tensor tvals,
    torch::Tensor error_flag,
    torch::Tensor gcursors,
    torch::Tensor ev_packed,
    torch::Tensor ev_vals,
    torch::Tensor ov_cursor,
    torch::Tensor ov_packed,
    torch::Tensor ov_vals,
    int64_t mode,
    int64_t region_bits,
    int64_t entry_w = ENTRY_W_CLASSIC) {
  int64_t nslots = tkeys.numel();
  int64_t nb = nslots >> region_bits;
  auto stream = at::hip::getCurrentHIPStream();
  uint64_t mask = (uint64_t)(nslots - 1);
  ScatterKind kind = scatter_kind_env();
  int coarse = scatter_coarse_bits(kind);
  int seg_bits = (int)region_bits + coarse;
  int64_t nseg = nslots >> seg_bits;
  size_t staged_lds = (size_t)nseg * SC_GRAN * 8 *
                          (mode == AGG_SUM ? 2 : 1) +
                      4 * (size_t)nseg * sizeof(int);
  while (kind == SCAT_STAGED &&
         (nseg < 1 || staged_lds > 160 * 1024 || seg_bits > 13)) {
    if (coarse > 0 && seg_bits > 13) {
      coarse -= 1;
    } else {
      kind = SCAT_FIXED;
      coarse = 0;
    }
    seg_bits = (int)region_bits + coarse;
    nseg = nslots >> seg_bits;
    staged_lds = (size_t)nseg * SC_GRAN * 8 * (mode == AGG_SUM ? 2 : 1) +
                 4 * (size_t)nseg * sizeof(int);
  }
  if (seg_bits > 13) {
    seg_bits = (int)region_bits;
    nseg = nb;
  }
  int64_t cap = ev_packed.numel() / nseg;
  if (kind == SCAT_STAGED) {
    cap &= ~(int64_t)(SC_GRAN - 1);
    if (cap < SC_GRAN) {
      kind = SCAT_FIXED;
      seg_bits = (int)region_bits;
      nseg = nb;
      cap = ev_packed.numel() / nseg;
    }
  }
  size_t agg_lds = (size_t)16 << seg_bits;
  dim3 agg_block(seg_bits >= 12 ? 1024 : 256);
  auto agg = [&](auto kern) {
    hipLaunchKernelGGL(
        kern, dim3((unsigned)nseg), agg_block, agg_lds, stream,
        (const uint64_t*)ev_packed.data_ptr<int64_t>(),
        mode == AGG_SUM ? ev_vals.data_ptr<int64_t>() : nullptr,
        gcursors.data_ptr<int32_t>(), cap,
        (uint64_t*)tkeys.data_ptr<int64_t>(),
        (unsigned long long*)tvals.data_ptr<int64_t>(), mask,
        (int)region_bits, seg_bits, error_flag.data_ptr<int32_t>());
  };
  if (mode == AGG_COUNT) {
    launch_count_agg(
        stream, (const uint64_t*)ev_packed.data_ptr<int64_t>(),
        gcursors.data_ptr<int32_t>(), cap,
        (uint64_t*)tkeys.data_ptr<int64_t>(),
        (unsigned long long*)tvals.data_ptr<int64_t>(), mask,
        (int)region_bits, seg_bits, nseg, error_flag.data_ptr<int32_t>(),
        mode == AGG_COUNT ? entry_w : ENTRY_W_CLASSIC);
  } else {
    agg(k_radix_agg<AGG_SUM>);
  }
  auto ov = [&](auto kern) {
    hipLaunchKernelGGL(
        kern, overflow_agg_grid(), dim3(256), 0, stream,
        (const uint64_t*)ov_packed.data_ptr<int64_t>(),
        mode == AGG_SUM ? ov_vals.data_ptr<int64_t>() : nullptr,
        ov_cursor.data_ptr<int32_t>(), ov_packed.numel(),
        (uint64_t*)tkeys.data_ptr<int64_t>(),
        (unsigned long long*)tvals.data_ptr<int64_t>(), mask,
        (int)region_bits, error_flag.data_ptr<int32_t>());
  };
  if (mode == AGG_COUNT) ov(k_overflow_agg<AGG_COUNT>);
  else ov(k_overflow_agg<AGG_SUM>);
}

void radix_v2_window_insert(
    torch::Tensor keys,
    torch::Tensor ts,
    torch::Tensor tkeys,
    torch::Tensor tvals,
    torch::Tensor max_ts,
    torch::Tensor error_flag,
    torch::Tensor gcur,
    torch::Tensor gres,
    torch::Tensor ev,
    torch::Tensor ev_res,
    int64_t align_ms,
    int64_t len_ms,
    int64_t ts_base,
    int64_t region_bits) {
  check_dev(keys, torch::kInt32, "keys");
  check_dev(ts, torch::kInt64, "ts");
  int64_t n = keys.numel();
  int64_t nslots = tkeys.numel();
  TORCH_CHECK((nslots & (nslots - 1)) == 0, "table size must be 2^k");
  int64_t cap_c = ev.numel() / V2_COARSE;
  TORCH_CHECK(cap_c % 8 == 0, "coarse capacity must be 8-aligned");
  int64_t res_cap = ev_res.numel() / V2_COARSE;
  if (n == 0) return;
  auto stream = at::hip::getCurrentHIPStream();
  uint64_t mask = (uint64_t)(nslots - 1);
  gcur.zero_();
  gres.zero_();
  hipLaunchKernelGGL(
      k_scatter_coarse, dim3(256), dim3(512), 0, stream,
      keys.data_ptr<int32_t>(), ts.data_ptr<int64_t>(), n, align_ms,
      len_ms, ts_base, mask, (int)region_bits, cap_c, res_cap,
      gcur.data_ptr<int32_t>(), gres.data_ptr<int32_t>(),
      (uint64_t*)ev.data_ptr<int64_t>(),
      (uint64_t*)ev_res.data_ptr<int64_t>(),
      (unsigned long long*)max_ts.data_ptr<int64_t>(),
      error_flag.data_ptr<int32_t>());
  int slices = 8;
  hipLaunchKernelGGL(
      k_agg_cached, dim3(V2_COARSE * slices), dim3(256), 0, stream,
      (const uint64_t*)ev.data_ptr<int64_t>(),
      (const uint64_t*)ev_res.data_ptr<int64_t>(),
      gcur.data_ptr<int32_t>(), gres.data_ptr<int32_t>(), cap_c, res_cap,
      slices, (uint64_t*)tkeys.data_ptr<int64_t>(),
      (unsigned long long*)tvals.data_ptr<int64_t>(), mask,
      (int)region_bits, error_flag.data_ptr<int32_t>());
}

static void launch_close_migrate(
    hipStream_t stream, const torch::Tensor& tkeys,
    const torch::Tensor& tvals, int64_t win_hi, const torch::Tensor& nkeys,
    const torch::Tensor& nvals, int64_t region_bits,
    const torch::Tensor& out_keys, const torch::Tensor& out_wins,
    const torch::Tensor& out_vals, const torch::Tensor& out_n,
    const torch::Tensor& error_flag) {
  int64_t nslots = tkeys.numel();
  int64_t nchunks = (nslots + CM_CHUNK - 1) / CM_CHUNK;
  if (nchunks < 1) nchunks = 1;
  unsigned grid = (unsigned)(nchunks < CM_MAX_GRID ? nchunks : CM_MAX_GRID);
  hipLaunchKernelGGL(
      k_close_migrate, dim3(grid), dim3(CM_BLK), 0, stream,
      (const uint64_t*)tkeys.data_ptr<int64_t>(),
      (const unsigned long long*)tvals.data_ptr<int64_t>(), nslots, win_hi,
      (uint64_t*)nkeys.data_ptr<int64_t>(),
      (unsigned long long*)nvals.data_ptr<int64_t>(),
      (uint64_t)(nslots - 1), (int)region_bits,
      out_keys.data_ptr<int32_t>(), out_wins.data_ptr<int32_t>(),
      out_vals.data_ptr<int64_t>(), out_n.data_ptr<int32_t>(),
      out_keys.numel(), error_flag.data_ptr<int32_t>());
}

int64_t close_extract(
    torch::Tensor tkeys,
    torch::Tensor tvals,
    int64_t win_lo,
    int64_t win_hi,
    torch::Tensor out_keys,
    torch::Tensor out_wins,
    torch::Tensor out_vals,
    torch::Tensor out_n) {
  check_dev(tkeys, torch::kInt64, "tkeys");
  check_dev(tvals, torch::kInt64, "tvals");
  check_dev(out_keys, torch::kInt32, "out_keys");
  check_dev(out_wins, torch::kInt32, "out_wins");
  check_dev(out_vals, torch::kInt64, "out_vals");
  check_dev(out_n, torch::kInt32, "out_n");
  int64_t nslots = tkeys.numel();
  auto stream = at::hip::getCurrentHIPStream();
  dim3 block(256);
  dim3 grid(n_blocks(nslots, 256));
  hipLaunchKernelGGL(
      k_close_extract, grid, block, 0, stream,
      (const uint64_t*)tkeys.data_ptr<int64_t>(),
      (const unsigned long long*)tvals.data_ptr<int64_t>(), nslots, win_lo,
      win_hi, out_keys.data_ptr<int32_t>(),
      out_wins.data_ptr<int32_t>(), out_vals.data_ptr<int64_t>(),
      out_n.data_ptr<int32_t>(), out_keys.numel());
  return 0;
}

void close_migrate(
    torch::Tensor tkeys,
    torch::Tensor tvals,
    torch::Tensor nkeys,
    torch::Tensor nvals,
    int64_t win_hi,
    int64_t region_bits,
    torch::Tensor out_keys,
    torch::Tensor out_wins,
    torch::Tensor out_vals,
    torch::Tensor out_n,
    torch::Tensor error_flag) {
  check_dev(tkeys, torch::kInt64, "tkeys");
  check_dev(nkeys, torch::kInt64, "nkeys");
  check_dev(tvals, torch::kInt64, "tvals");
  check_dev(nvals, torch::kInt64, "nvals");
  int64_t nslots = tkeys.numel();
  TORCH_CHECK(nkeys.numel() == nslots, "table size mismatch");
  launch_close_migrate(
      at::hip::getCurrentHIPStream(), tkeys, tvals, win_hi, nkeys, nvals,
      region_bits, out_keys, out_wins, out_vals, out_n, error_flag);
}

static void stats_insert_impl(
    torch::Tensor keys,
    torch::Tensor ts,
    torch::Tensor vals,
    torch::Tensor tkeys,
    torch::Tensor tcnt,
    torch::Tensor tsum,
    torch::Tensor tmin,
    torch::Tensor tmax,
    torch::Tensor max_ts,
    torch::Tensor error_flag,
    int64_t align_ms,
    int64_t len_ms,
    int64_t ts_base,
    const LateSink* late) {
  check_dev(keys, torch::kInt32, "keys");
  check_dev(ts, torch::kInt64, "ts");
  check_dev(vals, torch::kInt64, "vals");
  check_dev(tkeys, torch::kInt64, "tkeys");
  int64_t n = keys.numel();
  int64_t nslots = tkeys.numel();
  TORCH_CHECK((nslots & (nslots - 1)) == 0, "table size must be 2^k");
  if (n == 0) return;
  auto stream = at::hip::getCurrentHIPStream();
  dim3 block(256);
// ... 1398 lines not shown

  int64_t closed_horizon = closed_horizon_in;
  int64_t total_rows = 0;
  int pool = (int)key_pool.size();
  torch::Tensor cur_k = tkeys, cur_v = tvals;
  torch::Tensor alt_k = alt_tkeys, alt_v = alt_tvals;
  int swap_parity = 0;

  int* h_n = nullptr;
  HIP_CHECK(hipHostMalloc((void**)&h_n, sizeof(int), hipHostMallocDefault));

  bool pipe = pipelined && use_radix && !use_radix_v2 &&
              gcursors2.has_value();
  hipStream_t sc_stream = nullptr;
  hipEvent_t ev_sc[2] = {nullptr, nullptr};
  hipEvent_t ev_ag[2] = {nullptr, nullptr};
  int64_t nb = 0, cap = 0, nseg = 0;
  int seg_bits = (int)region_bits;
  ScatterKind kind = SCAT_FIXED;
  size_t staged_lds = 0;
  uint64_t mask = (uint64_t)(nslots - 1);
  uint64_t win_m2 = 0, win_maxfast = 0;
  if (pipe) {
    nb = nslots >> region_bits;
    TORCH_CHECK(ev_packed2->numel() == ev_packed->numel(),
                "pipelined scatter buffers must match");
    magic_div_u64(len_ms, &win_m2, &win_maxfast);
    kind = scatter_kind_env();
    int coarse = scatter_coarse_bits(kind);
    seg_bits = (int)region_bits + coarse;
    nseg = nslots >> seg_bits;
    staged_lds =
        (size_t)nseg * SC_GRAN * 8 + 4 * (size_t)nseg * sizeof(int);
    while (kind == SCAT_STAGED &&
           (nseg < 1 || staged_lds > 160 * 1024 || seg_bits > 13)) {
      if (coarse > 0 && seg_bits > 13) {
        coarse -= 1;
      } else {
        kind = SCAT_FIXED;
        coarse = 0;
      }
      seg_bits = (int)region_bits + coarse;
      nseg = nslots >> seg_bits;
      staged_lds =
          (size_t)nseg * SC_GRAN * 8 + 4 * (size_t)nseg * sizeof(int);
    }
    if (seg_bits > 13) {
      seg_bits = (int)region_bits;
      nseg = nb;
    }
    cap = ev_packed->numel() / nseg;
    if (kind == SCAT_STAGED) {
      cap &= ~(int64_t)(SC_GRAN - 1);
      if (cap < SC_GRAN) {
        kind = SCAT_FIXED;
        seg_bits = (int)region_bits;
        nseg = nb;
        cap = ev_packed->numel() / nseg;
      }
    }
    HIP_CHECK(hipStreamCreateWithFlags(&sc_stream, hipStreamNonBlocking));
    for (int i = 0; i < 2; ++i) {
      HIP_CHECK(hipEventCreateWithFlags(&ev_sc[i], hipEventDisableTiming));
      HIP_CHECK(hipEventCreateWithFlags(&ev_ag[i], hipEventDisableTiming));
    }
  }

  {
    pybind11::gil_scoped_release release;
    for (int64_t s = 0; s < n_steps; ++s) {
      if (step_ns != nullptr) {
        step_ns[s] = std::chrono::duration_cast<std::chrono::nanoseconds>(
                         std::chrono::steady_clock::now().time_since_epoch())
                         .count();
      }
      int64_t step = start_step + s;
      auto& keys = key_pool[step % pool];
      auto& ts = ts_pool[step % pool];
      int64_t base = align_ms + step * sim_ms_per_batch;
      if (use_radix_v2) {
        radix_v2_window_insert(
            keys, ts, cur_k, cur_v, max_ts, error_flag, *v2_gcur,
            *v2_gres, *v2_ev, *v2_ev_res, align_ms, len_ms, base,
            region_bits);
      } else if (pipe) {
        int par = (int)(step & 1);
        torch::Tensor& gcur = par ? *gcursors2 : *gcursors;
        torch::Tensor& evp = par ? *ev_packed2 : *ev_packed;
        torch::Tensor& ovc = par ? *ov_cursor2 : *ov_cursor;
        torch::Tensor& ovp = par ? *ov_packed2 : *ov_packed;
        if (s >= 2) {
          HIP_CHECK(hipStreamWaitEvent(sc_stream, ev_ag[par], 0));
        }
        HIP_CHECK(hipMemsetAsync(
            gcur.data_ptr<int32_t>(), 0, (size_t)nseg * sizeof(int),
            sc_stream));
        HIP_CHECK(hipMemsetAsync(
            ovc.data_ptr<int32_t>(), 0, sizeof(int), sc_stream));
        const CountEntries ce = plan_count_entries(
            kind == SCAT_STAGED, 1, evp.data_ptr<int64_t>(), nseg, cap,
            seg_bits, ts.scalar_type() == torch::kInt32, align_ms, len_ms,
            base);
        auto scat_step = [&](auto tsptr) {
          using TSV =
              std::remove_const_t<std::remove_pointer_t<decltype(tsptr)>>;
          if (kind == SCAT_STAGED) {
            launch_count_staged<TSV>(
                sc_stream, keys.data_ptr<int32_t>(), tsptr, n, 1, align_ms,
                len_ms, len_ms, base, mask, seg_bits, nseg, cap,
                gcur.data_ptr<int32_t>(), (uint64_t*)evp.data_ptr<int64_t>(),
                ovc.data_ptr<int32_t>(), (uint64_t*)ovp.data_ptr<int64_t>(),
                ovp.numel(), (unsigned long long*)max_ts.data_ptr<int64_t>(),
                error_flag.data_ptr<int32_t>(), win_m2, win_maxfast,
                true, ce);
          } else if (kind == SCAT_DIRECT) {
            hipLaunchKernelGGL(
                (k_radix_scatter_direct<AGG_COUNT, TSV>), grid, block, 0,
                sc_stream, keys.data_ptr<int32_t>(), tsptr,
                (const int64_t*)nullptr, n, align_ms, len_ms, len_ms, base,
                mask,
                seg_bits, cap, gcur.data_ptr<int32_t>(),
                (uint64_t*)evp.data_ptr<int64_t>(), (int64_t*)nullptr,
                ovc.data_ptr<int32_t>(), (uint64_t*)ovp.data_ptr<int64_t>(),
                (int64_t*)nullptr, ovp.numel(),
                (unsigned long long*)max_ts.data_ptr<int64_t>(),
                error_flag.data_ptr<int32_t>(), win_m2, win_maxfast);
          } else {
            size_t hist_lds = (size_t)nseg * sizeof(int);
            hipLaunchKernelGGL(
                (k_radix_scatter_fixed<AGG_COUNT, TSV>), grid, block,
                2 * hist_lds,
                sc_stream, keys.data_ptr<int32_t>(), tsptr,
                (const int64_t*)nullptr, n, align_ms, len_ms, len_ms, base, mask,
                seg_bits, cap, gcur.data_ptr<int32_t>(),
                (uint64_t*)evp.data_ptr<int64_t>(), (int64_t*)nullptr,
                ovc.data_ptr<int32_t>(), (uint64_t*)ovp.data_ptr<int64_t>(),
                (int64_t*)nullptr, ovp.numel(),
                (unsigned long long*)max_ts.data_ptr<int64_t>(),
                error_flag.data_ptr<int32_t>(), win_m2, win_maxfast,
                NO_LATE_ARGS);
          }
        };
        if (ts.scalar_type() == torch::kInt32)
          scat_step(ts.data_ptr<int32_t>());
        else scat_step(ts.data_ptr<int64_t>());
        HIP_CHECK(hipEventRecord(ev_sc[par], sc_stream));
        HIP_CHECK(hipStreamWaitEvent(stream, ev_sc[par], 0));
        launch_count_agg(
            stream, (const uint64_t*)evp.data_ptr<int64_t>(),
            gcur.data_ptr<int32_t>(), cap,
            (uint64_t*)cur_k.data_ptr<int64_t>(),
            (unsigned long long*)cur_v.data_ptr<int64_t>(), mask,
            (int)region_bits, seg_bits, nseg,
            error_flag.data_ptr<int32_t>(), ce.agg_w());
        hipLaunchKernelGGL(
            k_overflow_agg<AGG_COUNT>, overflow_agg_grid(), block, 0, stream,
            (const uint64_t*)ovp.data_ptr<int64_t>(),
            (const int64_t*)nullptr, ovc.data_ptr<int32_t>(), ovp.numel(),
            (uint64_t*)cur_k.data_ptr<int64_t>(),
            (unsigned long long*)cur_v.data_ptr<int64_t>(), mask,
            (int)region_bits, error_flag.data_ptr<int32_t>());
        HIP_CHECK(hipEventRecord(ev_ag[par], stream));
      } else if (use_radix) {
        radix_window_insert(
            keys, ts, c10::nullopt, cur_k, cur_v, max_ts, error_flag,
            *gcursors, *ev_packed, *ev_vals, *ov_cursor, *ov_packed,
            *ov_vals, align_ms, len_ms, AGG_COUNT, base, region_bits);
      } else {
        auto launch = [&](auto kern, auto tsptr) {
          hipLaunchKernelGGL(
              kern, grid, block, 0, stream, keys.data_ptr<int32_t>(),
              tsptr, (const int64_t*)nullptr, n,
              (uint64_t*)cur_k.data_ptr<int64_t>(),
              (unsigned long long*)cur_v.data_ptr<int64_t>(),
              (uint64_t)(nslots - 1), align_ms, len_ms, len_ms, base,
              (int)region_bits,
              (unsigned long long*)max_ts.data_ptr<int64_t>(),
              error_flag.data_ptr<int32_t>(), (const int64_t*)nullptr,
              NO_LATE_ARGS);
        };
        auto disp = [&](auto tsptr) {
          using TSV =
              std::remove_const_t<std::remove_pointer_t<decltype(tsptr)>>;
          if (dedup)
            launch(k_window_agg_insert<AGG_COUNT, true, TSV>, tsptr);
          else launch(k_window_agg_insert<AGG_COUNT, false, TSV>, tsptr);
        };
        if (ts.scalar_type() == torch::kInt32)
          disp(ts.data_ptr<int32_t>());
        else disp(ts.data_ptr<int64_t>());
      }

      int64_t wm = base + sim_ms_per_batch - 1;
      int64_t horizon = (wm - wait_ms - align_ms) / len_ms;
      if (horizon > closed_horizon) {
        HIP_CHECK(hipMemsetAsync(out_n.data_ptr<int32_t>(), 0, sizeof(int), stream));
        launch_close_migrate(
            stream, cur_k, cur_v, horizon, alt_k, alt_v, region_bits,
            out_keys, out_wins, out_vals, out_n, error_flag);
        HIP_CHECK(hipMemcpyAsync(h_n, out_n.data_ptr<int32_t>(), sizeof(int),
                       hipMemcpyDeviceToHost, stream));
        std::swap(cur_k, alt_k);
        std::swap(cur_v, alt_v);
        swap_parity ^= 1;
        HIP_CHECK(hipMemsetAsync(alt_k.data_ptr<int64_t>(), 0xFF,
                                 (size_t)nslots * 8, stream));
        HIP_CHECK(hipMemsetAsync(alt_v.data_ptr<int64_t>(), 0,
                                 (size_t)nslots * 8, stream));
        HIP_CHECK(hipStreamSynchronize(stream));
        total_rows += *h_n;
        closed_horizon = horizon;
      }
    }
    if (sc_stream != nullptr) {
      HIP_CHECK(hipStreamSynchronize(sc_stream));
    }
    HIP_CHECK(hipStreamSynchronize(stream));
  }
  if (sc_stream != nullptr) {
    for (int i = 0; i < 2; ++i) {
      HIP_CHECK(hipEventDestroy(ev_sc[i]));
      HIP_CHECK(hipEventDestroy(ev_ag[i]));
    }
    HIP_CHECK(hipStreamDestroy(sc_stream));
  }
  HIP_CHECK(hipHostFree(h_n));
  auto* st = state_out.data_ptr<int64_t>();
  st[0] = closed_horizon;
  st[1] = total_rows;
  st[2] = swap_parity;
  return total_rows;
}

int64_t native_run_window_steps_graph(
    std::vector<torch::Tensor> key_pool,
    std::vector<torch::Tensor> ts_pool,
    int64_t start_step,
    int64_t n_steps,
    int64_t sim_ms_per_batch,
    torch::Tensor tkeys,
    torch::Tensor tvals,
    torch::Tensor max_ts,
    torch::Tensor error_flag,
    torch::Tensor out_keys,
    torch::Tensor out_wins,
    torch::Tensor out_vals,
    torch::Tensor out_n,
    int64_t align_ms,
    int64_t len_ms,
    int64_t wait_ms,
    int64_t closed_horizon_in,
    torch::Tensor state_out,
    int64_t region_bits,
    torch::Tensor alt_tkeys,
    torch::Tensor alt_tvals,
    torch::Tensor ts_base_dev) {
  TORCH_CHECK(!key_pool.empty(), "empty key pool");
  int64_t nslots = tkeys.numel();
  TORCH_CHECK((nslots & (nslots - 1)) == 0, "table size must be 2^k");
  int64_t n = key_pool[0].numel();
  auto stream = at::hip::getCurrentHIPStream();
  dim3 block(256);
  dim3 grid(n_blocks(n, 256));
  int pool = (int)key_pool.size();
  uint64_t mask = (uint64_t)(nslots - 1);

  ts_base_dev.fill_(align_ms + start_step * sim_ms_per_batch);

  auto launch_insert_on = [&](int j, hipStream_t st) {
    hipLaunchKernelGGL(
        (k_window_agg_insert<AGG_COUNT, false>), grid, block, 0, st,
        key_pool[j].data_ptr<int32_t>(), ts_pool[j].data_ptr<int64_t>(),
        (const int64_t*)nullptr, n, (uint64_t*)tkeys.data_ptr<int64_t>(),
        (unsigned long long*)tvals.data_ptr<int64_t>(), mask, align_ms,
        len_ms, len_ms, 0, (int)region_bits,
        (unsigned long long*)max_ts.data_ptr<int64_t>(),
        error_flag.data_ptr<int32_t>(),
        (const int64_t*)ts_base_dev.data_ptr<int64_t>(), NO_LATE_ARGS);
    hipLaunchKernelGGL(
        k_bump, dim3(1), dim3(1), 0, st,
        ts_base_dev.data_ptr<int64_t>(), sim_ms_per_batch);
  };
  auto launch_insert = [&](int j) { launch_insert_on(j, stream); };

  int64_t closed_horizon = closed_horizon_in;
  int64_t total_rows = 0;
  int* h_n = nullptr;
  HIP_CHECK(hipHostMalloc((void**)&h_n, sizeof(int), hipHostMallocDefault));

  hipGraph_t graph = nullptr;
  hipGraphExec_t gexec = nullptr;
  {
    pybind11::gil_scoped_release release;
    hipStream_t cs = nullptr;
    HIP_CHECK(hipStreamCreateWithFlags(&cs, hipStreamNonBlocking));
    HIP_CHECK(hipStreamBeginCapture(cs, hipStreamCaptureModeThreadLocal));
    for (int j = 0; j < pool; ++j) launch_insert_on(j, cs);
    HIP_CHECK(hipStreamEndCapture(cs, &graph));
    HIP_CHECK(hipStreamDestroy(cs));
    HIP_CHECK(hipGraphInstantiate(&gexec, graph, nullptr, nullptr, 0));

    auto horizon_after = [&](int64_t step) {
      int64_t wm = align_ms + (step + 1) * sim_ms_per_batch - 1;
      return (wm - wait_ms - align_ms) / len_ms;
    };
    auto do_close = [&](int64_t horizon) {
      HIP_CHECK(hipMemsetAsync(out_n.data_ptr<int32_t>(), 0, sizeof(int),
                               stream));
      launch_close_migrate(
          stream, tkeys, tvals, horizon, alt_tkeys, alt_tvals, region_bits,
          out_keys, out_wins, out_vals, out_n, error_flag);
      HIP_CHECK(hipMemcpyAsync(h_n, out_n.data_ptr<int32_t>(), sizeof(int),
                               hipMemcpyDeviceToHost, stream));
      HIP_CHECK(hipMemsetAsync(tkeys.data_ptr<int64_t>(), 0xFF,
// ... 165 lines not shown
      ov_vals.data_ptr<int64_t>(), ov_cursor.data_ptr<int32_t>(),
      ov_packed.numel(), (uint64_t*)skeys.data_ptr<int64_t>(),
      (long long*)sstart.data_ptr<int64_t>(),
      (long long*)slast.data_ptr<int64_t>(),
      (long long*)sacc.data_ptr<int64_t>(), mask, gap_ms,
      out_keys.data_ptr<int32_t>(), out_start.data_ptr<int64_t>(),
      out_end.data_ptr<int64_t>(), out_vals.data_ptr<int64_t>(),
      out_n.data_ptr<int32_t>(), out_keys.numel(),
      error_flag.data_ptr<int32_t>());
}


int64_t dict_encode(
    torch::Tensor bytes,
    torch::Tensor offs,
    torch::Tensor dlo,
    torch::Tensor dhi,
    torch::Tensor dids,
    torch::Tensor counter,
    torch::Tensor new_ids,
    torch::Tensor new_idx,
    torch::Tensor new_n,
    torch::Tensor out_ids,
    torch::Tensor error_flag) {
  check_dev(bytes, torch::kUInt8, "bytes");
  check_dev(offs, torch::kInt64, "offs");
  check_dev(dlo, torch::kInt64, "dlo");
  check_dev(out_ids, torch::kInt32, "out_ids");
  int64_t n = offs.numel() - 1;
  int64_t nslots = dlo.numel();
  TORCH_CHECK((nslots & (nslots - 1)) == 0, "dict size must be 2^k");
  if (n == 0) return 0;
  auto stream = at::hip::getCurrentHIPStream();
  dim3 block(256);
  dim3 grid(n_blocks(n, 256));
  uint64_t mask = (uint64_t)(nslots - 1);
  new_n.zero_();
  hipLaunchKernelGGL(
      k_dict_insert, grid, block, 0, stream,
      bytes.data_ptr<uint8_t>(), offs.data_ptr<int64_t>(), n,
      (uint64_t*)dlo.data_ptr<int64_t>(),
      (uint64_t*)dhi.data_ptr<int64_t>(), dids.data_ptr<int32_t>(), mask,
      counter.data_ptr<int32_t>(), new_ids.data_ptr<int32_t>(),
      new_idx.data_ptr<int32_t>(), new_n.data_ptr<int32_t>(),
      new_ids.numel(), error_flag.data_ptr<int32_t>());
  hipLaunchKernelGGL(
      k_dict_lookup, grid, block, 0, stream,
      bytes.data_ptr<uint8_t>(), offs.data_ptr<int64_t>(), n,
      (const uint64_t*)dlo.data_ptr<int64_t>(),
      (const uint64_t*)dhi.data_ptr<int64_t>(), dids.data_ptr<int32_t>(),
      mask, out_ids.data_ptr<int32_t>(), error_flag.data_ptr<int32_t>());
  return n;
}

void dict_restore(
    torch::Tensor bytes,
    torch::Tensor offs,
    torch::Tensor ids,
    torch::Tensor dlo,
    torch::Tensor dhi,
    torch::Tensor dids,
    torch::Tensor error_flag) {
  check_dev(bytes, torch::kUInt8, "bytes");
  check_dev(offs, torch::kInt64, "offs");
  check_dev(ids, torch::kInt32, "ids");
  int64_t n = offs.numel() - 1;
  int64_t nslots = dlo.numel();
  TORCH_CHECK((nslots & (nslots - 1)) == 0, "dict size must be 2^k");
  if (n == 0) return;
  auto stream = at::hip::getCurrentHIPStream();
  hipLaunchKernelGGL(
      k_dict_insert_pinned, dim3(n_blocks(n, 256)), dim3(256), 0, stream,
      bytes.data_ptr<uint8_t>(), offs.data_ptr<int64_t>(),
      ids.data_ptr<int32_t>(), n, (uint64_t*)dlo.data_ptr<int64_t>(),
      (uint64_t*)dhi.data_ptr<int64_t>(), dids.data_ptr<int32_t>(),
      (uint64_t)(nslots - 1), error_flag.data_ptr<int32_t>());
}

void str_exchange_pack(
    torch::Tensor bytes,
    torch::Tensor offs,
    torch::Tensor ts,
    c10::optional<torch::Tensor> vals,
    int64_t world,
    torch::Tensor counts,
    torch::Tensor byte_counts,
    torch::Tensor send_lens,
    torch::Tensor send_ts,
    torch::Tensor send_vals,
    torch::Tensor send_bytes
) {
  check_dev(bytes, torch::kUInt8, "bytes");
  check_dev(offs, torch::kInt64, "offs");
  check_dev(ts, torch::kInt64, "ts");
  check_dev(send_lens, torch::kInt32, "send_lens");
  int64_t n = offs.numel() - 1;
  TORCH_CHECK(world >= 1, "world must be >= 1");
  TORCH_CHECK(send_lens.numel() >= n, "send_lens too small");
  TORCH_CHECK(send_bytes.numel() >= bytes.numel(), "send_bytes too small");
  counts.zero_();
  byte_counts.zero_();
  if (n == 0) return;
  auto stream = at::hip::getCurrentHIPStream();
  dim3 block(256);
  dim3 grid(n_blocks(n, 256));
  hipLaunchKernelGGL(
      k_str_bucket_hist, grid, block, 0, stream,
      bytes.data_ptr<uint8_t>(), offs.data_ptr<int64_t>(), n, (int)world,
      counts.data_ptr<int32_t>(),
      (long long*)byte_counts.data_ptr<int64_t>());
  auto cursors =
      (torch::cumsum(counts, 0, torch::kInt32) - counts).contiguous();
  const int64_t* vptr =
      vals.has_value() ? vals->data_ptr<int64_t>() : nullptr;
  auto src_idx = torch::empty(
      {n}, torch::TensorOptions()
               .dtype(torch::kInt32)
               .device(bytes.device()));
  hipLaunchKernelGGL(
      k_str_meta_scatter, grid, block, 0, stream,
      bytes.data_ptr<uint8_t>(), offs.data_ptr<int64_t>(),
      ts.data_ptr<int64_t>(), vptr, n, (int)world,
      cursors.data_ptr<int32_t>(), send_lens.data_ptr<int32_t>(),
      send_ts.data_ptr<int64_t>(),
      vptr != nullptr ? send_vals.data_ptr<int64_t>() : nullptr,
      src_idx.data_ptr<int32_t>());
  auto lens64 = send_lens.narrow(0, 0, n).to(torch::kInt64);
  auto send_offs = (torch::cumsum(lens64, 0) - lens64).contiguous();
  hipLaunchKernelGGL(
      k_str_byte_gather, grid, block, 0, stream,
      bytes.data_ptr<uint8_t>(), offs.data_ptr<int64_t>(),
      src_idx.data_ptr<int32_t>(), send_offs.data_ptr<int64_t>(), n,
      send_bytes.data_ptr<uint8_t>());
}

PYBIND11_MODULE(TORCH_EXTENSION_NAME, m) {
  m.def("str_exchange_pack", &str_exchange_pack,
        "pack a str batch into per-rank wire segments (content-hash "
        "owner) for the all-to-allv string exchange");
  m.def("session_radix_insert", &session_radix_insert,
        "fused radix session insert: AGG_TS scatter + per-segment LDS "
        "session aggregation + sequential overflow walk");
  m.def("dict_encode", &dict_encode,
        "device string-dictionary encode: 2-phase insert+lookup");
  m.def("dict_restore", &dict_restore,
        "device string-dictionary restore with pinned ids");
  m.def("window_agg_insert", &window_agg_insert,
        "Fused window-id + hash-insert + watermark over an event batch");
  m.def("radix_v2_window_insert", &radix_v2_window_insert,
        "Experimental two-level radix with full-line LDS-staged "
        "scatter (COUNT mode)");
  m.def("radix_scatter_only", &radix_scatter_only,
        "Scatter stage of the radix insert on the current stream; returns "
        "the entry base for radix_agg_only");
  m.def("radix_agg_only", &radix_agg_only,
        "Aggregation stage of the radix insert on the current stream",
        pybind11::arg("tkeys"), pybind11::arg("tvals"),
        pybind11::arg("error_flag"), pybind11::arg("gcursors"),
        pybind11::arg("ev_packed"), pybind11::arg("ev_vals"),
        pybind11::arg("ov_cursor"), pybind11::arg("ov_packed"),
        pybind11::arg("ov_vals"), pybind11::arg("mode"),
        pybind11::arg("region_bits"),
        pybind11::arg("entry_w") = (int64_t)ENTRY_W_CLASSIC);
  m.def("window_agg_insert_late", &window_agg_insert_late,
        "Single-pass window insert that diverts events below the late "
        "cutoff to a late buffer");
  m.def("radix_window_insert_late", &radix_window_insert_late,
        "Radix window insert that diverts events below the late cutoff "
        "to a late buffer");
  m.def("stats_insert_late", &stats_insert_late,
        "Stats insert that diverts events below the late cutoff to a "
        "late buffer");
  m.def("radix_stats_insert_late", &radix_stats_insert_late,
        "Radix stats insert that diverts events below the late cutoff "
        "to a late buffer");
  m.def("radix_window_insert", &radix_window_insert,
        "Radix-partitioned LDS-staged keyed window aggregation");
  m.def("close_migrate", &close_migrate,
        "Window close with reclamation: emit closed cells and migrate "
        "live cells into a fresh table");
  m.def("close_extract", &close_extract,
        "Extract (and clear) closed windows from the keyed state table");
  m.def("stats_insert", &stats_insert,
        "Keyed running count/sum/min/max over an event batch (1BRC)");
  m.def("radix_stats_insert", &radix_stats_insert,
        "Radix-partitioned LDS-staged keyed stats aggregation");
  m.def("stats_fixup", &stats_fixup,
        "Add count/sum deltas to existing stats slots (recovery)");
  m.def("stats_extract", &stats_extract,
        "Extract (and clear) keyed stats below a window horizon");
  m.def("stats_close_migrate", &stats_close_migrate,
        "Stats close with reclamation: emit due cells, migrate live "
        "cells into a fresh table, drop cells below the closed horizon");
  m.def("stats_pane_close", &stats_pane_close,
        "Sliding stats close: fold the panes of due windows into a fold "
        "table, migrate live panes into a fresh table, drop dead panes");
  m.def("radix_join_insert", &radix_join_insert,
        "Region-partitioned stream join insert (L2-local table ops)");
  m.def("join_insert", &join_insert,
        "Stream-stream hash join insert; emits completed pairs");
  m.def("session_insert", &session_insert,
        "Gap-based session aggregation over a (key, ts)-sorted batch");
  m.def("session_close_migrate", &session_close_migrate,
        "Emit sessions idle past the horizon; migrate live cells");
  m.def("session_restore", &session_restore,
        "Rebuild session cells from a host spill");
  m.def("session_run_collapse", &session_run_collapse,
        "Collapse a (key, ts)-sorted batch into gap-separated runs");
  m.def("session_run_merge", &session_run_merge,
        "Merge sorted runs into the multi-session table (also restore)");
  m.def("session_multi_close_migrate", &session_multi_close_migrate,
        "Emit each cell's closable prefix; migrate the open sessions");
  m.def("session_merge_batch", &session_merge_batch,
        "Merge per-key per-batch (count, min_ts, max_ts) rows into "
        "the session table (gap >= batch span fast path)");
  m.def("join_extract", &join_extract,
        "Extract live join state (recovery snapshot)");
  m.def("filter_compact", &filter_compact,
        "Stream compaction of a RecordBatch by a boolean mask");
  m.def("bucket_hist", &bucket_hist, "Per-destination counts for exchange");
  m.def("bucket_scatter", &bucket_scatter,
        "Scatter events into per-destination segments for all-to-allv");
  m.def("native_run_window_steps_graph", &native_run_window_steps_graph,
        "hipGraph-captured native step loop (latency mode: one graph "
        "launch per pool cycle)");
  m.def("native_run_window_steps", &native_run_window_steps,
        "Run N steps of the columnar window pipeline with no Python "
        "between steps (native step loop)");
}
```

### bytewax_amd/gpu/__init__.py

```python

from dataclasses import dataclass
from datetime import datetime, timezone
from typing import Any, Dict, Optional, Tuple

from ._ext import build as build_ext
from ._ext import ext

EPOCH_UTC = datetime(1970, 1, 1, tzinfo=timezone.utc)

AGG_COUNT = 0
AGG_SUM = 1

_INT64_MAX = (1 << 63) - 1


def _ms(dt: datetime) -> int:
    return int((dt - EPOCH_UTC).total_seconds() * 1000)


@dataclass
class RecordBatch:

    keys: Any
    ts: Any
    vals: Optional[Any] = None
    max_ts: Optional[int] = None
    ts_base: int = 0

    def __len__(self) -> int:
        return int(self.keys.numel())


def _mix64_np(x):
    import numpy as np

    x = x ^ (x >> np.uint64(33))
    x = x * np.uint64(0xFF51AFD7ED558CCD)
    x = x ^ (x >> np.uint64(33))
    x = x * np.uint64(0xC4CEB9FE1A85EC53)
    x = x ^ (x >> np.uint64(33))
    return x


def key_owner(keys, world: int):
    import numpy as np
    import torch

    if world < 1:
        msg = f"world must be >= 1, got {world}"
        raise ValueError(msg)
    if keys.dtype != torch.int32:
        msg = f"key_owner takes int32 keys, got {keys.dtype}"
        raise TypeError(msg)
    k = keys.detach().cpu().contiguous().numpy()
    h = _mix64_np(k.view(np.uint32).astype(np.uint64))
    return torch.from_numpy((h % np.uint64(world)).astype(np.int64))


def _bucket_cpu(batch: RecordBatch, world: int):
    import torch

    dst = key_owner(batch.keys, world)
    order = torch.argsort(dst, stable=True)
    counts = torch.bincount(dst, minlength=world).to(torch.int32)
    send_keys = batch.keys[order]
    send_ts = batch.ts[order]
    send_vals = batch.vals[order] if batch.vals is not None else None
    return counts, send_keys, send_ts, send_vals


def exchange_by_key(
    batch: RecordBatch, group=None, async_op: bool = False,
    force: bool = False,
):
    import torch
    import torch.distributed as dist

    world = dist.get_world_size(group)
    if world == 1 and not force:
        return ([], batch) if async_op else batch
    dev = batch.keys.device
    n = len(batch)
    has_vals = batch.vals is not None
    if dev.type == "cpu":
        counts, send_keys, send_ts, send_vals = _bucket_cpu(batch, world)
    else:
        k = ext()
        counts = torch.zeros(world, dtype=torch.int32, device=dev)
        k.bucket_hist(batch.keys, world, counts)
        offsets = torch.cumsum(counts, 0, dtype=torch.int32) - counts
        cursors = offsets.clone()
        send_keys = torch.empty(n, dtype=torch.int32, device=dev)
        send_ts = torch.empty(n, dtype=batch.ts.dtype, device=dev)
        send_vals = torch.empty(
            n if has_vals else 0, dtype=torch.int64, device=dev
        )
        k.bucket_scatter(
            batch.keys,
            batch.ts,
            batch.vals if has_vals else None,
            world,
            cursors,
            send_keys,
            send_ts,
            send_vals,
        )
    recv_counts = torch.empty_like(counts)
    dist.all_to_all_single(recv_counts, counts, group=group)
    in_splits = counts.tolist()
    out_splits = recv_counts.tolist()
    m = int(sum(out_splits))

    if batch.ts.dtype == torch.int32:
        ts_base = batch.ts_base
        send_ts32 = send_ts
    elif batch.max_ts is not None:
        ts_base = batch.max_ts - (1 << 30)
        send_ts32 = (send_ts - (ts_base - batch.ts_base)).to(torch.int32)
    else:
        ts_base = (
            int(send_ts.min().item()) + batch.ts_base if n > 0 else 0
        )
        send_ts32 = (send_ts - (ts_base - batch.ts_base)).to(torch.int32)
    bases = torch.zeros(world, dtype=torch.int64, device=dev)
    my_base = torch.full((world,), ts_base, dtype=torch.int64, device=dev)
    dist.all_to_all_single(bases, my_base, group=group)

    recv_keys = torch.empty(m, dtype=torch.int32, device=dev)
    recv_ts32 = torch.empty(m, dtype=torch.int32, device=dev)
    works = []
    w = dist.all_to_all_single(
        recv_keys, send_keys, out_splits, in_splits, group=group,
        async_op=async_op,
    )
    if w is not None:
        works.append(w)
    w = dist.all_to_all_single(
        recv_ts32, send_ts32, out_splits, in_splits, group=group,
        async_op=async_op,
    )
    if w is not None:
        works.append(w)
    recv_vals = None
    if has_vals:
        recv_vals = torch.empty(m, dtype=torch.int64, device=dev)
        w = dist.all_to_all_single(
            recv_vals, send_vals, out_splits, in_splits, group=group,
            async_op=async_op,
        )
        if w is not None:
            works.append(w)
    out = _LazyTsBatch(
        recv_keys, recv_ts32, out_splits, bases.tolist(), recv_vals,
        batch.max_ts,
    )
    if async_op:
        return (works, out)
    return out.materialize()


class _LazyTsBatch:

    def __init__(self, keys, ts32, seg_counts, seg_bases, vals, max_ts):
        self.keys = keys
# ... 105 lines not shown
        if 2 * self.bound <= self.cap:
            return
        if self._probe_pin is None:
            self._probe_pin = torch.zeros(
                1, dtype=torch.int32, pin_memory=True
            )
        self._probe_pin.copy_(self.n, non_blocking=True)
        ev = torch.cuda.Event()
        ev.record()
        self._probe = (ev, self._probe_pin)
        self._since_probe = 0

    def drain(self, error_flag) -> None:
        if self.cpu:
            self.carry.extend(self.pending)
            self.pending = []
            self.bound = 0
            return
        if self.n is None or self.bound == 0:
            return
        import torch

        n, flag = torch.cat([self.n, error_flag]).tolist()
        _check_error_flag(flag & ERR_LATE_OVERFLOW, "late buffer")
        if n > self.cap:
            msg = f"late cursor {n} past late_cap {self.cap}"
            raise RuntimeError(msg)
        if n:
            self.carry.append(
                (
                    self.keys[:n].clone(),
                    self.ts[:n].clone(),
                    self.vals[:n].clone() if self.has_vals else None,
                )
            )
            self.n.zero_()
        self.bound = 0

    def add_host(self, keys, ts, vals) -> None:
        if len(keys):
            self.pending.append((keys, ts, vals if self.has_vals else None))

    def take(self, error_flag) -> Optional["RecordBatch"]:
        import torch

        self.drain(error_flag)
        if not self.carry:
            return None
        chunks, self.carry = self.carry, []
        keys = torch.cat([c[0] for c in chunks])
        ts = torch.cat([c[1] for c in chunks])
        vals = torch.cat([c[2] for c in chunks]) if self.has_vals else None
        return RecordBatch(keys, ts, vals)


def _split_late_cpu(batch: "RecordBatch", cutoff: int, late: _LateTracker):
    import torch

    late.reserve(len(batch), None)
    abs_ts = batch.ts.to(torch.int64) + batch.ts_base
    is_late = abs_ts < cutoff
    if not bool(is_late.any()):
        return batch
    late.add_host(
        batch.keys[is_late],
        abs_ts[is_late],
        batch.vals[is_late] if batch.vals is not None else None,
    )
    keep = ~is_late
    return RecordBatch(
        batch.keys[keep],
        batch.ts[keep],
        batch.vals[keep] if batch.vals is not None else None,
        max_ts=batch.max_ts,
        ts_base=batch.ts_base,
    )


class WindowAggState:

    def __init__(
        self,
        device,
        align_ms: int,
        len_ms: int,
        mode: int = AGG_COUNT,
        slots_pow: int = 20,
        dedup: bool = False,
        out_cap: int = 1 << 20,
        radix: bool = False,
        region_bits: int = 11,
        max_batch: int = 0,
        off_ms: int = 0,
        radix_v2: bool = False,
        track_late: bool = False,
        wait_ms: int = 0,
        late_cap: int = 0,
    ):
        import torch

        if track_late and (dedup or radix_v2):
            msg = "track_late is incompatible with dedup and radix_v2"
            raise ValueError(msg)
        self.track_late = track_late
        self.wait_ms = wait_ms
        self._late = (
            _LateTracker(device, wait_ms, mode == AGG_SUM, late_cap)
            if track_late
            else None
        )

        self.device = device
        self.align_ms = align_ms
        self.len_ms = len_ms
        self.off_ms = off_ms if off_ms > 0 else len_ms
        if self.off_ms > len_ms:
            msg = "window offset must be <= length"
            raise ValueError(msg)
        if self.off_ms < len_ms and dedup:
            msg = "sliding windows are incompatible with the dedup path"
            raise ValueError(msg)
        self.expand = (
            -(-len_ms // self.off_ms) if self.off_ms < len_ms else 1
        )
        self.mode = mode
        self.dedup = dedup
        self.max_ts_host = 0
        self.closed_horizon = -(1 << 62)
        self._close_pending = False
        self._close_ev = None
        self._outn_pin = None
        self._carry_cpu = None
        if radix_v2 and (mode != AGG_COUNT or dedup):
            msg = "radix_v2 supports the COUNT mode only"
            raise ValueError(msg)
        self.radix_v2 = radix_v2 and device.type != "cpu"
        if self.radix_v2:
            radix = True
        self.radix = radix
        self.region_bits = region_bits if radix else 0
        self.cpu = device.type == "cpu"
        if radix and not self.cpu:
            self.n_regions = (1 << slots_pow) >> region_bits
            if self.n_regions < 1:
                msg = "slots_pow must exceed region_bits"
                raise ValueError(msg)
            self.rx_gcursors = torch.zeros(
                self.n_regions, dtype=torch.int32, device=device
            )
            self.rx_ov_cursor = torch.zeros(
                1, dtype=torch.int32, device=device
            )
            self._alloc_rx(max(max_batch, 1))
        if self.cpu:
            self._table: Dict[Tuple[int, int], int] = {}
            return
        self.k = ext()
        self.nslots = 1 << slots_pow
        self.tkeys = torch.full(
            (self.nslots,), -1, dtype=torch.int64, device=device
        )
        self.tvals = torch.zeros(self.nslots, dtype=torch.int64, device=device)
        self.tkeys_alt = torch.full(
            (self.nslots,), -1, dtype=torch.int64, device=device
        )
        self.tvals_alt = torch.zeros(
            self.nslots, dtype=torch.int64, device=device
        )
        self.max_ts_dev = torch.zeros(1, dtype=torch.int64, device=device)
        self.error_flag = torch.zeros(1, dtype=torch.int32, device=device)
        self.out_cap = out_cap
        self.out_keys = torch.empty(out_cap, dtype=torch.int32, device=device)
        self.out_wins = torch.empty(out_cap, dtype=torch.int32, device=device)
        self.out_vals = torch.empty(out_cap, dtype=torch.int64, device=device)
        self.out_n = torch.zeros(1, dtype=torch.int32, device=device)
        self._pin_keys = None

    def _insert_cpu(self, batch: RecordBatch) -> None:
        import numpy as np

        if self.track_late:
            batch = _split_late_cpu(
                batch, self.max_ts_host - self.wait_ms, self._late
            )
        keys = batch.keys.numpy()
        ts64 = batch.ts.numpy().astype("int64", copy=False)
        wins = (
            (ts64 + batch.ts_base - self.align_ms) // self.off_ms
        ).astype("int64")
        if self.mode == AGG_COUNT:
            vals = np.ones(len(keys), dtype="int64")
        else:
            vals = batch.vals.numpy()
        packed = (wins << 32) | keys.astype("uint32")
        uniq, inv = np.unique(packed, return_inverse=True)
        sums = np.bincount(inv, weights=vals).astype("int64")
        for p, s in zip(uniq.tolist(), sums.tolist()):
            kw = (int(np.uint32(p & 0xFFFFFFFF)), int(p >> 32))
            self._table[kw] = self._table.get(kw, 0) + s
        if self.off_ms < self.len_ms:
            t_arr = batch.ts.numpy().astype("int64", copy=False) + batch.ts_base
            lo = (t_arr - self.align_ms - self.len_ms) // self.off_ms + 1
            for k, w_hi, w_lo, v in zip(
                keys.tolist(), wins.tolist(), lo.tolist(), vals.tolist()
            ):
                for wn in range(int(w_lo), int(w_hi)):
                    kw = (int(k), int(wn))
                    self._table[kw] = self._table.get(kw, 0) + int(v)
        mx = int(batch.ts.max().item()) + batch.ts_base if len(batch) else 0
        if mx > self.max_ts_host:
            self.max_ts_host = mx

    def _alloc_rx(self, max_batch: int) -> None:
        import torch

        per_region = max(
            32,
            -(-max_batch * self.expand * 5 // 2) // self.n_regions + 1,
        )
        total = per_region * self.n_regions
        self.rx_max_batch = max_batch
        self.rx_packed = torch.empty(
            total, dtype=torch.int64, device=self.device
        )
        if getattr(self, "radix_v2", False):
            cap_c = (-(-max_batch * 5 // 2) // 256 + 8) // 8 * 8
            res_cap = max(1 << 14, cap_c // 4)
            self.v2_gcur = torch.zeros(256, dtype=torch.int32, device=self.device)
            self.v2_gres = torch.zeros(256, dtype=torch.int32, device=self.device)
            self.v2_ev = torch.empty(
                256 * cap_c, dtype=torch.int64, device=self.device
            )
            self.v2_ev_res = torch.empty(
                256 * res_cap, dtype=torch.int64, device=self.device
            )
        self.rx_vals = torch.empty(
            total if self.mode == AGG_SUM else 0,
            dtype=torch.int64,
            device=self.device,
        )
        ov = max(1 << 20, max_batch)
        self.rx_ov_packed = torch.empty(
            ov, dtype=torch.int64, device=self.device
        )
        self.rx_ov_vals = torch.empty(
            ov if self.mode == AGG_SUM else 0,
            dtype=torch.int64,
            device=self.device,
        )
        if hasattr(self, "rx_packed2"):
            self.rx_gcursors2 = torch.zeros_like(self.rx_gcursors)
            self.rx_packed2 = torch.empty_like(self.rx_packed)
            self.rx_vals2 = torch.empty_like(self.rx_vals)
            self.rx_ov_cursor2 = torch.zeros_like(self.rx_ov_cursor)
            self.rx_ov_packed2 = torch.empty_like(self.rx_ov_packed)
            self.rx_ov_vals2 = torch.empty_like(self.rx_ov_vals)

    def insert(self, batch: RecordBatch) -> None:
        if self.cpu:
            self._insert_cpu(batch)
            if (
                batch.max_ts is not None
                and batch.max_ts > self.max_ts_host
            ):
                self.max_ts_host = batch.max_ts
            return
        if self.radix and len(batch) > self.rx_max_batch:
            self._alloc_rx(int(len(batch) * 5 // 4))
        import torch

        if self.track_late:
            self._insert_late(batch)
            return
        if self.radix_v2:
            self.k.radix_v2_window_insert(
                batch.keys,
                batch.ts.to(torch.int64),
                self.tkeys,
                self.tvals,
                self.max_ts_dev,
                self.error_flag,
                self.v2_gcur,
                self.v2_gres,
                self.v2_ev,
                self.v2_ev_res,
                self.align_ms,
                self.len_ms,
                batch.ts_base,
                self.region_bits,
            )
        elif self.radix:
            self.k.radix_window_insert(
                batch.keys,
                batch.ts,
                batch.vals,
                self.tkeys,
                self.tvals,
                self.max_ts_dev,
                self.error_flag,
                self.rx_gcursors,
                self.rx_packed,
                self.rx_vals,
                self.rx_ov_cursor,
                self.rx_ov_packed,
                self.rx_ov_vals,
                self.align_ms,
                self.len_ms,
                self.mode,
                batch.ts_base,
                self.region_bits,
                self.off_ms,
                [],
                [],
            )
        else:
            self.k.window_agg_insert(
                batch.keys,
                batch.ts,
                batch.vals,
                self.tkeys,
                self.tvals,
                self.max_ts_dev,
                self.error_flag,
                self.align_ms,
                self.len_ms,
                self.mode,
                self.dedup,
                batch.ts_base,
                self.region_bits,
                self.off_ms,
            )
        if batch.max_ts is not None and batch.max_ts > self.max_ts_host:
            self.max_ts_host = batch.max_ts

    def _insert_late(self, batch: RecordBatch) -> None:
        lt = self._late
        lt.reserve(len(batch), self.error_flag)
        cutoff = self.max_ts_host - self.wait_ms
        late_args = (cutoff, lt.keys, lt.ts, lt.vals, lt.n)
        if self.radix:
            self.k.radix_window_insert_late(
                batch.keys,
                batch.ts,
                batch.vals,
                self.tkeys,
                self.tvals,
                self.max_ts_dev,
                self.error_flag,
                self.rx_gcursors,
                self.rx_packed,
                self.rx_vals,
                self.rx_ov_cursor,
                self.rx_ov_packed,
                self.rx_ov_vals,
                self.align_ms,
                self.len_ms,
                self.mode,
                batch.ts_base,
                self.region_bits,
                self.off_ms,
                *late_args,
            )
        else:
            self.k.window_agg_insert_late(
                batch.keys,
                batch.ts,
                batch.vals,
                self.tkeys,
                self.tvals,
                self.max_ts_dev,
                self.error_flag,
                self.align_ms,
                self.len_ms,
                self.mode,
                batch.ts_base,
                self.region_bits,
                self.off_ms,
                *late_args,
            )
        lt.inserted()
        if batch.max_ts is not None:
            if batch.max_ts > self.max_ts_host:
                self.max_ts_host = batch.max_ts
        else:
            self.watermark_ms(sync=True)

    def take_late(self) -> Optional[RecordBatch]:
        if self._late is None:
            return None
        return self._late.take(None if self.cpu else self.error_flag)

    def late_drained(self) -> bool:
        return self._late is not None and bool(self._late.carry)

    def _ordered_only(self, what: str) -> None:
        if self.track_late:
            msg = f"{what} is watermark-ordered only; track_late needs insert()"
            raise ValueError(msg)

    def _ensure_pipe(self) -> None:
        import torch

        if getattr(self, "_pipe_ready", False):
            return
        self._pipe_ready = True
        self._sc_stream = torch.cuda.Stream(self.device)
        self._pipe_parity = 0
        self._ev_sc = [torch.cuda.Event(), torch.cuda.Event()]
        self._ev_w = [None, None]
        self._ev_ag = [torch.cuda.Event(), torch.cuda.Event()]
        self._ag_recorded = [False, False]
        if not hasattr(self, "rx_packed2"):
            self.rx_gcursors2 = torch.zeros_like(self.rx_gcursors)
            self.rx_packed2 = torch.empty_like(self.rx_packed)
            self.rx_vals2 = torch.empty_like(self.rx_vals)
            self.rx_ov_cursor2 = torch.zeros_like(self.rx_ov_cursor)
            self.rx_ov_packed2 = torch.empty_like(self.rx_ov_packed)
            self.rx_ov_vals2 = torch.empty_like(self.rx_ov_vals)

    def _pipe_bufs(self, par: int):
        if par == 0:
            return (
                self.rx_gcursors,
                self.rx_packed,
                self.rx_vals,
                self.rx_ov_cursor,
                self.rx_ov_packed,
                self.rx_ov_vals,
            )
        return (
            self.rx_gcursors2,
            self.rx_packed2,
            self.rx_vals2,
            self.rx_ov_cursor2,
            self.rx_ov_packed2,
            self.rx_ov_vals2,
        )

    def insert_pipelined(
        self,
        keys,
        ts,
        vals,
        ts_base: int,
        seg_counts,
        seg_bases,
        max_ts: Optional[int],
        works=None,
    ) -> None:
        self._ordered_only("insert_pipelined")
        import torch

        n = int(keys.numel())
        if n > self.rx_max_batch:
            if getattr(self, "_pipe_ready", False):
                torch.cuda.synchronize(self.device)
            self._alloc_rx(int(n * 5 // 4))
        self._ensure_pipe()
        par = self._pipe_parity
        self._pipe_parity ^= 1
        bufs = self._pipe_bufs(par)
        cur = torch.cuda.current_stream(self.device)
        with torch.cuda.stream(self._sc_stream):
            if works:
                for w in works:
                    w.wait()
            if self._ag_recorded[par]:
                self._sc_stream.wait_event(self._ev_ag[par])
            keys.record_stream(self._sc_stream)
            ts.record_stream(self._sc_stream)
            if vals is not None:
                vals.record_stream(self._sc_stream)
            self._ev_w[par] = self.k.radix_scatter_only(
                keys,
                ts,
                vals,
                self.max_ts_dev,
                self.error_flag,
                *bufs,
                self.nslots,
                self.align_ms,
                self.len_ms,
                self.mode,
                ts_base,
                self.region_bits,
                self.off_ms,
                list(seg_counts),
                [int(b) for b in seg_bases],
            )
            self._ev_sc[par].record(self._sc_stream)
        cur.wait_event(self._ev_sc[par])
        self.k.radix_agg_only(
            self.tkeys,
            self.tvals,
            self.error_flag,
            *bufs,
            self.mode,
            self.region_bits,
            self._ev_w[par],
        )
        self._ev_ag[par].record(cur)
        self._ag_recorded[par] = True
        if max_ts is not None and max_ts > self.max_ts_host:
            self.max_ts_host = max_ts

    def insert_lazy(self, lz: "_LazyTsBatch") -> None:
        self._ordered_only("insert_lazy")
        if self.cpu or not self.radix or self.radix_v2:
            self.insert(lz.materialize())
            return
        n = len(lz)
        if n > self.rx_max_batch:
            self._alloc_rx(int(n * 5 // 4))
        self.k.radix_window_insert(
            lz.keys,
            lz.ts32,
            lz.vals,
            self.tkeys,
            self.tvals,
            self.max_ts_dev,
            self.error_flag,
            self.rx_gcursors,
            self.rx_packed,
            self.rx_vals,
            self.rx_ov_cursor,
            self.rx_ov_packed,
            self.rx_ov_vals,
            self.align_ms,
            self.len_ms,
            self.mode,
            0,
            self.region_bits,
            self.off_ms,
            lz.seg_counts,
            lz.seg_bases,
        )
        if lz.max_ts is not None and lz.max_ts > self.max_ts_host:
            self.max_ts_host = lz.max_ts

    def watermark_ms(self, sync: bool = False) -> int:
        if sync and not self.cpu:
            dev = int(self.max_ts_dev.item())
            if dev > self.max_ts_host:
                self.max_ts_host = dev
        return self.max_ts_host

    def _extract_cpu(
        self, win_lo: int, win_hi: int, delete: bool
    ) -> Optional[RecordBatch]:
        import torch

        hit = [
            (k, w, v)
            for (k, w), v in self._table.items()
            if win_lo <= w < win_hi
        ]
        if not hit:
            return None
        if delete:
            for k, w, _v in hit:
                del self._table[(k, w)]
        keys = torch.tensor([k for k, _w, _v in hit], dtype=torch.int32)
        ts = torch.tensor(
            [w * self.off_ms + self.align_ms for _k, w, _v in hit],
            dtype=torch.int64,
        )
        vals = torch.tensor([v for _k, _w, v in hit], dtype=torch.int64)
        return RecordBatch(keys, ts, vals)

    def _read_out(self) -> Optional[RecordBatch]:
        import torch

        n = int(self.out_n.item())
        if n > self.out_cap:
            msg = (
                f"window close produced {n} rows > out_cap {self.out_cap}; "
                "increase out_cap"
            )
            raise RuntimeError(msg)
        _check_error_flag(
            int(self.error_flag.item()), "keyed window state table"
        )
        if n == 0:
            return None
        return RecordBatch(
            self.out_keys[:n].clone(),
            self.out_wins[:n].to(torch.int64) * self.off_ms + self.align_ms,
            self.out_vals[:n].clone(),
        )

    def _extract_range(self, win_lo: int, win_hi: int) -> Optional[RecordBatch]:
        if self.cpu:
            return self._extract_cpu(win_lo, win_hi, delete=False)
        self.out_n.zero_()
        self.k.close_extract(
            self.tkeys,
            self.tvals,
            win_lo,
            win_hi,
            self.out_keys,
            self.out_wins,
            self.out_vals,
            self.out_n,
        )
        return self._read_out()

    def close_due(self, wait_ms: int = 0) -> Optional[RecordBatch]:
        wm = self.watermark_ms()
        horizon = (
            wm - wait_ms - self.align_ms - self.len_ms
        ) // self.off_ms + 1
        if horizon <= self.closed_horizon:
            return None
        if self.cpu:
            out = self._extract_cpu(-(1 << 40), horizon, delete=True)
            self.closed_horizon = horizon
            return out
        self.out_n.zero_()
        self.k.close_migrate(
            self.tkeys,
            self.tvals,
            self.tkeys_alt,
            self.tvals_alt,
            horizon,
            self.region_bits,
            self.out_keys,
            self.out_wins,
            self.out_vals,
            self.out_n,
            self.error_flag,
        )
        self.tkeys, self.tkeys_alt = self.tkeys_alt, self.tkeys
        self.tvals, self.tvals_alt = self.tvals_alt, self.tvals
        self.tkeys_alt.fill_(-1)
        self.tvals_alt.zero_()
        out = self._read_out()
        self.closed_horizon = horizon
        return out

    def close_launch(self, wait_ms: int = 0) -> None:
        import torch

        if self._close_pending:
            return
        wm = self.watermark_ms()
        horizon = (
            wm - wait_ms - self.align_ms - self.len_ms
        ) // self.off_ms + 1
        if horizon <= self.closed_horizon:
            return
        if self.cpu:
            self._carry_cpu = self._extract_cpu(
                -(1 << 40), horizon, delete=True
            )
            self.closed_horizon = horizon
            self._close_pending = self._carry_cpu is not None
            return
        self.out_n.zero_()
        self.k.close_migrate(
            self.tkeys,
            self.tvals,
            self.tkeys_alt,
            self.tvals_alt,
            horizon,
            self.region_bits,
            self.out_keys,
            self.out_wins,
            self.out_vals,
            self.out_n,
            self.error_flag,
        )
        self.tkeys, self.tkeys_alt = self.tkeys_alt, self.tkeys
        self.tvals, self.tvals_alt = self.tvals_alt, self.tvals
        self.tkeys_alt.fill_(-1)
        self.tvals_alt.zero_()
        self.closed_horizon = horizon
        if self._outn_pin is None:
            self._outn_pin = torch.zeros(
                2,
                dtype=torch.int32,
                pin_memory=torch.cuda.is_available(),
            )
        self._outn_pin[0:1].copy_(self.out_n, non_blocking=True)
        self._outn_pin[1:2].copy_(self.error_flag, non_blocking=True)
        self._close_ev = torch.cuda.Event()
        self._close_ev.record()
        self._close_pending = True

    def close_resolve(self) -> Optional[RecordBatch]:
        import torch

        if not self._close_pending:
            return None
        self._close_pending = False
        if self.cpu:
            out = self._carry_cpu
            self._carry_cpu = None
            return out
        self._close_ev.synchronize()
        n = int(self._outn_pin[0].item())
        _check_error_flag(
            int(self._outn_pin[1].item()), "keyed window state table"
        )
        if n > self.out_cap:
            msg = (
                f"window close produced {n} rows > out_cap "
                f"{self.out_cap}; increase out_cap"
            )
            raise RuntimeError(msg)
        if n == 0:
            return None
        return RecordBatch(
            self.out_keys[:n].clone(),
            self.out_wins[:n].to(torch.int64) * self.off_ms + self.align_ms,
            self.out_vals[:n].clone(),
        )

    def close_all(self) -> Optional[RecordBatch]:
        if self._close_pending:
            msg = "close_resolve() the pending close before close_all()"
            raise RuntimeError(msg)
        if self.cpu:
            return self._extract_cpu(self.closed_horizon, 1 << 40, delete=True)
        out = self._extract_range(self.closed_horizon, 1 << 40)
        self.closed_horizon = 1 << 40
        return out

    def snapshot_to_host(self) -> Dict[str, Any]:
        import torch

        if self.cpu:
            import numpy as np

            items = list(self._table.items())
            return {
                "keys": np.array([k for (k, _w), _v in items], dtype="int32"),
                "wins": np.array([w for (_k, w), _v in items], dtype="int32"),
                "vals": np.array([v for _kw, v in items], dtype="int64"),
                "max_ts": self.watermark_ms(),
                "closed_horizon": self.closed_horizon,
            }
        self.out_n.zero_()
        self.k.close_extract(
            self.tkeys,
            self.tvals,
            self.closed_horizon,
            1 << 40,
            self.out_keys,
            self.out_wins,
            self.out_vals,
            self.out_n,
        )
        n = int(self.out_n.item())
        if self._pin_keys is None or self._pin_keys.numel() < n:
            cap = max(n, 1)
            pin = torch.cuda.is_available()
            self._pin_keys = torch.empty(cap, dtype=torch.int32, pin_memory=pin)
            self._pin_wins = torch.empty(cap, dtype=torch.int32, pin_memory=pin)
            self._pin_vals = torch.empty(cap, dtype=torch.int64, pin_memory=pin)
        self._pin_keys[:n].copy_(self.out_keys[:n], non_blocking=True)
        self._pin_wins[:n].copy_(self.out_wins[:n], non_blocking=True)
        self._pin_vals[:n].copy_(self.out_vals[:n], non_blocking=True)
        if torch.cuda.is_available():
            torch.cuda.synchronize(self.device)
        return {
            "keys": self._pin_keys[:n].numpy().copy(),
            "wins": self._pin_wins[:n].numpy().copy(),
            "vals": self._pin_vals[:n].numpy().copy(),
            "max_ts": self.watermark_ms(),
            "closed_horizon": self.closed_horizon,
        }

    def native_run(
        self,
        key_pool,
        ts_pool,
        start_step: int,
        n_steps: int,
        sim_ms_per_batch: int,
        wait_ms: int = 0,
        pipelined: bool = True,
    ):
        self._ordered_only("native_run")
        import torch

        if self.cpu:
            msg = "native_run requires a device table"
            raise RuntimeError(msg)
        pipe = pipelined and self.radix and not self.radix_v2
        if pipe and not hasattr(self, "rx_gcursors2"):
            self.rx_gcursors2 = torch.zeros_like(self.rx_gcursors)
            self.rx_packed2 = torch.empty_like(self.rx_packed)
            self.rx_ov_cursor2 = torch.zeros_like(self.rx_ov_cursor)
            self.rx_ov_packed2 = torch.empty_like(self.rx_ov_packed)
        step_ns = torch.zeros(n_steps, dtype=torch.int64)
        state_out = torch.zeros(3, dtype=torch.int64)
        rows = self.k.native_run_window_steps(
            list(key_pool),
            list(ts_pool),
            start_step,
            n_steps,
            sim_ms_per_batch,
            self.tkeys,
            self.tvals,
            self.max_ts_dev,
            self.error_flag,
            self.out_keys,
            self.out_wins,
            self.out_vals,
            self.out_n,
            self.align_ms,
            self.len_ms,
            wait_ms,
            self.mode,
            self.dedup,
            self.closed_horizon,
            step_ns,
            state_out,
            self.region_bits,
            self.radix,
            self.rx_gcursors if self.radix else None,
            self.rx_packed if self.radix else None,
            self.rx_vals if self.radix else None,
            self.rx_ov_cursor if self.radix else None,
            self.rx_ov_packed if self.radix else None,
            self.rx_ov_vals if self.radix else None,
            self.tkeys_alt,
            self.tvals_alt,
            self.radix_v2,
            self.v2_gcur if self.radix_v2 else None,
            self.v2_gres if self.radix_v2 else None,
            self.v2_ev if self.radix_v2 else None,
            self.v2_ev_res if self.radix_v2 else None,
            pipe,
            self.rx_gcursors2 if pipe else None,
            self.rx_packed2 if pipe else None,
            self.rx_ov_cursor2 if pipe else None,
            self.rx_ov_packed2 if pipe else None,
        )
        if int(state_out[2].item()) == 1:
            self.tkeys, self.tkeys_alt = self.tkeys_alt, self.tkeys
            self.tvals, self.tvals_alt = self.tvals_alt, self.tvals
        self.closed_horizon = int(state_out[0].item())
        self.max_ts_host = max(
            self.max_ts_host,
            self.align_ms + (start_step + n_steps) * sim_ms_per_batch - 1,
        )
        if int(self.error_flag.item()) != 0:
            msg = "keyed window state table overflowed; increase slots_pow"
            raise RuntimeError(msg)
        return rows, step_ns

# ... 128 lines not shown
```

Baseline: 122.6 billion events/s.

## Add compact 4-byte radix scatter entries via invertible key/window mixing

Adds a compact entry format for COUNT-mode radix insert. The window delta and key are packed into 32+dbits bits, scrambled with an invertible mixing function, and the high bits are used as the segment index, so each scatter entry drops from 8 bytes to 4. New compact scatter and aggregation kernels write and read these 32-bit entries, and the aggregation kernel counts in 32-bit LDS cells, roughly halving scatter/agg memory traffic. A spill counter is also added: if overflow spills exceed a set share of inserted events since the last close, the host falls back to 8-byte hashed entries. The trade-off is extra hash/unhash arithmetic per event and a narrower window range, since events outside it go to the slower overflow path.

```diff
diff --git a/bytewax_amd/_native/stream_kernels.hip b/bytewax_amd/_native/stream_kernels.hip
--- a/bytewax_amd/_native/stream_kernels.hip
+++ b/bytewax_amd/_native/stream_kernels.hip
@@ -525,6 +525,57 @@
 __device__ __forceinline__ uint64_t entry_classic(
     uint64_t entry, uint32_t wlo) {
   return ((uint64_t)(wlo + entry_delta(entry)) << 32) | (entry >> 32);
+}
+
+#define ENTRY_PAD32 0xFFFFFFFFu
+#define ENTRY_FMT_CLASSIC 0
+#define ENTRY_FMT_HASHED 1
+#define ENTRY_FMT_COMPACT 2
+#define MIXN_C1 0xff51afd7ed558ccdULL
+#define MIXN_C2 0xc4ceb9fe1a85ec53ULL
+#define MIXN_C3 0x9e3779b97f4a7c15ULL
+
+constexpr uint64_t mixn_inverse_of(uint64_t c) {
+  uint64_t x = c;
+  for (int i = 0; i < 6; ++i) x *= 2 - c * x;
+  return x;
+}
+
+__host__ __device__ __forceinline__ uint64_t mixn(uint64_t x, int n) {
+  const uint64_t m = ((uint64_t)1 << n) - 1;
+  const int s = (n + 1) >> 1;
+  x ^= x >> s;
+  x = (x * MIXN_C1) & m;
+  x ^= x >> s;
+  x = (x * MIXN_C2) & m;
+  x ^= x >> s;
+  x = (x * MIXN_C3) & m;
+  x ^= x >> s;
+  return x;
+}
+
+__host__ __device__ __forceinline__ uint64_t mixn_inv(uint64_t y, int n) {
+  const uint64_t m = ((uint64_t)1 << n) - 1;
+  const int s = (n + 1) >> 1;
+  constexpr uint64_t i1 = mixn_inverse_of(MIXN_C1);
+  constexpr uint64_t i2 = mixn_inverse_of(MIXN_C2);
+  constexpr uint64_t i3 = mixn_inverse_of(MIXN_C3);
+  static_assert(i1 * MIXN_C1 == 1 && i2 * MIXN_C2 == 1 && i3 * MIXN_C3 == 1,
+                "inverse constants");
+  y ^= y >> s;
+  y = (y * i3) & m;
+  y ^= y >> s;
+  y = (y * i2) & m;
+  y ^= y >> s;
+  y = (y * i1) & m;
+  y ^= y >> s;
+  return y;
+}
+
+__device__ __forceinline__ uint64_t compact_classic(
+    uint32_t seg, uint32_t e, int n, uint32_t wbase) {
+  uint64_t x = mixn_inv(((uint64_t)seg << 31) | e, n);
+  return ((uint64_t)(wbase + (uint32_t)(x >> 32)) << 32) | (uint32_t)x;
 }
 
 template <int MODE, typename TS = int64_t, bool LATE = false>
@@ -1155,6 +1206,218 @@
   }
 }
 
+#define SCC_GRAN 16
+#define GDC_SPILL 0x80000000u
+
+static inline size_t compact_lds_bytes(int64_t nseg, int64_t tile) {
+  size_t stage_n = (size_t)(tile + (SCC_GRAN - 1) * nseg);
+  return stage_n * 4
+         + (size_t)nseg * SCC_GRAN * 4
+         + 3 * (size_t)nseg * sizeof(int)
+         + (stage_n / SCC_GRAN) * sizeof(uint32_t);
+}
+
+template <int U = 16, int BLK = 512>
+__global__ __launch_bounds__(BLK) void k_radix_scatter_compact(
+    const int32_t* __restrict__ keys,
+    const int32_t* __restrict__ ts,
+    int64_t n,
+    int64_t align_ms,
+    int64_t len_ms,
+    int64_t ts_base,
+    int dbits,
+    int64_t cap,
+    int* __restrict__ gcursors,
+    uint32_t* __restrict__ ev32,
+    int* __restrict__ ov_cursor,
+    uint64_t* __restrict__ ov_packed,
+    int64_t ov_cap,
+    unsigned long long* __restrict__ max_ts,
+    int* __restrict__ error_flag,
+    uint64_t win_m2,
+    uint64_t win_maxfast,
+    Win32 w32) {
+  constexpr int T = BLK * U;
+  constexpr int NW = BLK / WAVE;
+  static_assert(T + (SCC_GRAN - 1) * BLK < (1 << 14),
+                "staging offset must fit 14 bits");
+  static_assert(T <= (1 << 13), "tile rank shares a word with the segment");
+  extern __shared__ __attribute__((aligned(16))) char smem_cc[];
+  __shared__ int s_wtot[NW];
+  const int nseg = 2 << dbits;
+  const int nbits = 32 + dbits;
+  const uint32_t dlimit = 1u << dbits;
+  const uint32_t wbase = w32.wlo + w32.qoff;
+  const int stage_n = T + (SCC_GRAN - 1) * nseg;
+  uint32_t* stage = (uint32_t*)smem_cc;
+  uint32_t* res = stage + stage_n;
+  int* res_cnt = (int*)(res + (size_t)nseg * SCC_GRAN);
+  int* lhist = res_cnt + nseg;
+  uint32_t* lpack = (uint32_t*)(lhist + nseg);
+  uint32_t* gdst = lpack + nseg;
+  const int tid = threadIdx.x;
+  const int lane = tid & (WAVE - 1);
+  const int wave = tid / WAVE;
+  if (tid < nseg) {
+    res_cnt[tid] = 0;
+    lhist[tid] = 0;
+  }
+  __syncthreads();
+
+  auto spill = [&](uint64_t packed) {
+    int opos = atomicAdd(ov_cursor, 1);
+    if (opos < ov_cap) ov_packed[opos] = packed;
+    else atomicOr(error_flag, 1);
+  };
+
+  int32_t rk[U];
+  int32_t rt[U];
+  auto load_tile = [&](int64_t t0) {
+#pragma unroll
+    for (int u = 0; u < U; ++u) {
+      int64_t i = t0 + u * BLK + tid;
+      if (i > n - 1) i = n - 1;
+      rk[u] = keys[i];
+      rt[u] = ts[i];
+    }
+  };
+  const int64_t stride = (int64_t)gridDim.x * T;
+  int64_t local_max = 0;
+  int64_t t0 = (int64_t)blockIdx.x * T;
+  const bool seen = t0 + tid < n;
+  if (t0 < n) {
+    load_tile(t0);
+    local_max = (int64_t)rt[0];
+  }
+  for (; t0 < n; t0 += stride) {
+    uint32_t pk[U];
+    int sr[U];
+    int64_t left64 = n - t0 - tid;
+    const int left = left64 > T ? T : (left64 < 0 ? 0 : (int)left64);
+    int32_t dmax = (int32_t)local_max;
+    uint32_t rare = 0;
+#pragma unroll
+    for (int u = 0; u < U; ++u) {
+      const bool in = u * BLK < left;
+      const uint32_t d = (uint32_t)rt[u];
+      const uint32_t q = win32_div(d + w32.c, w32);
+      const uint32_t delta = q - w32.qoff;
+      const bool fits = d - w32.dlo < w32.dspan && delta < dlimit;
+      const uint64_t y = mixn(
+          ((uint64_t)(delta & (dlimit - 1)) << 32) | (uint32_t)rk[u], nbits);
+      pk[u] = (uint32_t)y & 0x7FFFFFFFu;
+      if (in && !fits) rare |= 1u << u;
+      if (in && (int32_t)d > dmax) dmax = (int32_t)d;
+      const bool ok = in && fits;
+      int b = (int)(y >> 31);
+      int rank = atomicAdd(&lhist[b], ok ? 1 : 0);
+      sr[u] = ok ? ((rank << 13) | b) : -1;
+    }
+    local_max = dmax;
+    while (rare != 0) {
+      int u = __ffs(rare) - 1;
+      rare &= rare - 1;
+      int64_t i = t0 + u * BLK + tid;
+      int64_t win = win_of((int64_t)ts[i] + ts_base, align_ms, len_ms,
+                           win_m2, win_maxfast);
+      spill(((uint64_t)(uint32_t)(int32_t)win << 32) | (uint32_t)keys[i]);
+    }
+    if (t0 + stride < n) load_tile(t0 + stride);
+    __syncthreads();
+    int rc = 0, grant = 0, gb = 0;
+    if (tid < nseg) {
+      rc = res_cnt[tid];
+      int tot = rc + lhist[tid];
+      grant = tot & ~(SCC_GRAN - 1);
+      if (grant > 0) gb = atomicAdd(&gcursors[tid], grant);
+      res_cnt[tid] = tot - grant;
+      lhist[tid] = 0;
+    }
+    int incl = grant;
+    for (int o = 1; o < WAVE; o <<= 1) {
+      int v = __shfl_up(incl, o);
+      if (lane >= o) incl += v;
+    }
+    if (lane == WAVE - 1) s_wtot[wave] = incl;
+    __syncthreads();
+    int total = 0, woff = 0;
+    for (int w = 0; w < NW; ++w) {
+      int v = s_wtot[w];
+      if (w < wave) woff += v;
+      total += v;
+    }
+    const int off = woff + incl - grant;
+    if (wave * WAVE < nseg) {
+      const int og = grant > 0 ? off : -1;
+      for (int k = 0; k < WAVE / 4; ++k) {
+        const int src = k * 4 + (lane >> 4);
+        const int o = __shfl(og, src);
+        const int j = lane & (SCC_GRAN - 1);
+        if (o >= 0 && j < SCC_GRAN - 1)
+          stage[o + j] = res[(size_t)(wave * WAVE + src) * SCC_GRAN + j];
+      }
+    }
+    if (tid < nseg) {
+      lpack[tid] = (uint32_t)off | ((uint32_t)rc << 14) |
+                   ((uint32_t)grant << 18);
+      if (grant > 0) {
+        for (int j = 0; j < grant; j += SCC_GRAN) {
+          int64_t gp = (int64_t)gb + j;
+          gdst[(off + j) / SCC_GRAN] =
+              gp < cap ? (uint32_t)(((int64_t)tid * cap + gp) / SCC_GRAN)
+                       : (GDC_SPILL | (uint32_t)tid);
+        }
+      }
+    }
+    __syncthreads();
+    for (int u = 0; u < U; ++u) {
+      if (sr[u] < 0) continue;
+      int b = sr[u] & ((1 << 13) - 1);
+      uint32_t w = lpack[b];
+      int vpos = (int)((w >> 14) & 15u) + (sr[u] >> 13);
+      int g = (int)(w >> 18);
+      if (vpos < g) stage[(w & ((1u << 14) - 1)) + vpos] = pk[u];
+      else res[(size_t)b * SCC_GRAN + (vpos - g)] = pk[u];
+    }
+    __syncthreads();
+    for (int p = tid; p < total / 4; p += BLK) {
+      uint4 v = *(const uint4*)(stage + 4 * p);
+      uint32_t d = gdst[p / 4];
+      if ((d & GDC_SPILL) == 0) {
+        *(uint4*)(ev32 + (int64_t)d * SCC_GRAN + 4 * (p & 3)) = v;
+      } else {
+        const uint32_t seg = d & ~GDC_SPILL;
+        const uint32_t e[4] = {v.x, v.y, v.z, v.w};
+        for (int j = 0; j < 4; ++j)
+          if (e[j] != ENTRY_PAD32)
+            spill(compact_classic(seg, e[j], nbits, wbase));
+      }
+    }
+  }
+  __syncthreads();
+  if (tid < nseg) {
+    int rc = res_cnt[tid];
+    if (rc > 0) {
+      int gb = atomicAdd(&gcursors[tid], SCC_GRAN);
+      for (int j = 0; j < SCC_GRAN; ++j) {
+        uint32_t e = j < rc ? res[(size_t)tid * SCC_GRAN + j] : ENTRY_PAD32;
+        int64_t gp = (int64_t)gb + j;
+        if (gp < cap) ev32[(int64_t)tid * cap + gp] = e;
+        else if (e != ENTRY_PAD32)
+          spill(compact_classic((uint32_t)tid, e, nbits, wbase));
+      }
+    }
+  }
+  local_max = seen ? local_max + ts_base : 0;
+  for (int off = WAVE / 2; off > 0; off >>= 1) {
+    int64_t other = __shfl_down((long long)local_max, off);
+    if (other > local_max) local_max = other;
+  }
+  if ((threadIdx.x & (WAVE - 1)) == 0 && local_max > 0) {
+    atomicMax(max_ts, (unsigned long long)local_max);
+  }
+}
+
 template <int MODE>
 __global__ void k_overflow_agg(
     const uint64_t* __restrict__ ov_packed,
@@ -1165,9 +1428,12 @@
     unsigned long long* __restrict__ tvals,
     uint64_t mask,
     int region_bits,
-    int* __restrict__ error_flag) {
+    int* __restrict__ error_flag,
+    unsigned long long* __restrict__ spill_total) {
   int64_t n = *ov_cursor;
   if (n > ov_cap) n = ov_cap;
+  if (spill_total != nullptr && blockIdx.x == 0 && threadIdx.x == 0 && n > 0)
+    *spill_total += (unsigned long long)n;
   int64_t i = blockIdx.x * (int64_t)blockDim.x + threadIdx.x;
   int64_t stride = gridDim.x * (int64_t)blockDim.x;
   for (; i < n; i += stride) {
@@ -1469,6 +1735,164 @@
       uint64_t packed = ((uint64_t)win << 32) | (c >> 32);
       if (!hash_add(tkeys, tvals, mask, region_bits, packed,
                     c & 0x0FFFFFFFULL)) {
+        atomicOr(error_flag, 1);
+      }
+    }
+  }
+}
+
+template <int BLK, int R>
+__global__ __launch_bounds__(BLK, BLK == 1024 ? 8 : 4) void k_radix_agg_compact(
+    const uint32_t* __restrict__ ev32,
+    const int* __restrict__ counts,
+    int64_t cap,
+    uint64_t* __restrict__ tkeys,
+    unsigned long long* __restrict__ tvals,
+    uint64_t mask,
+    int region_bits,
+    int lds_bits,
+    int* __restrict__ error_flag,
+    uint32_t wbase,
+    int dbits) {
+  extern __shared__ char smem[];
+  unsigned long long* cells = (unsigned long long*)smem;
+  const int region = 1 << lds_bits;
+  const uint32_t lmask = (uint32_t)region - 1;
+  const int sshift = 31 - lds_bits;
+  const int nbits = 32 + dbits;
+  const int b = blockIdx.x;
+  int cnt = counts[b];
+  if (cnt > (int)cap) cnt = (int)cap;
+  if (cnt <= 0) return;
+  for (int s = threadIdx.x; s < region / 2; s += BLK) {
+    ((agg_u64x2*)cells)[s] = agg_u64x2{EMPTY_SLOT, EMPTY_SLOT};
+  }
+  const uint32_t* seg = ev32 + (int64_t)b * cap;
+  __syncthreads();
+
+  auto escape = [&](uint32_t e) {
+    if (!hash_add(tkeys, tvals, mask, region_bits,
+                  compact_classic((uint32_t)b, e, nbits, wbase), 1ULL)) {
+      atomicOr(error_flag, 1);
+    }
+  };
+  auto drain = [&](uint32_t pend, auto entry, auto start, auto skipped) {
+    uint32_t tag = 0;
+    uint32_t lh = 0;
+    int left = 0;
+    while (left != 0 || pend != 0) {
+      if (left == 0) {
+        int e = __ffs(pend) - 1;
+        pend &= pend - 1;
+        tag = entry(e);
+        lh = start(e);
+        left = region - (skipped(e) ? 1 : 0);
+      }
+      unsigned long long cur = cells[lh];
+      if (cur == EMPTY_SLOT) {
+        cur = atomicCAS(&cells[lh], EMPTY_SLOT,
+                        (unsigned long long)tag << 32);
+        if (cur == EMPTY_SLOT) cur = (unsigned long long)tag << 32;
+      }
+      if ((uint32_t)(cur >> 32) == tag) {
+        atomicAdd((unsigned int*)&cells[lh], 1u);
+        left = 0;
+      } else {
+        lh = (lh + 1) & lmask;
+        if (--left == 0) escape(tag);
+      }
+    }
+  };
+  auto add_one = [&](uint32_t e) {
+    if (e == ENTRY_PAD32) return;
+    drain(
+        1u, [&](int) { return e; }, [&](int) { return e >> sshift; },
+        [&](int) { return false; });
+  };
+
+  int head = (int)(((16 - ((uintptr_t)seg & 15)) & 15) >> 2);
+  if (head > cnt) head = cnt;
+  const int nvec = (cnt - head) >> 2;
+  const int tail = head + 4 * nvec;
+  if (threadIdx.x == 0)
+    for (int j = 0; j < head; ++j) add_one(seg[j]);
+  if (threadIdx.x == BLK - 1)
+    for (int j = tail; j < cnt; ++j) add_one(seg[j]);
+
+  const uint4* vseg = (const uint4*)(seg + head);
+  constexpr int chunk = R * BLK;
+  constexpr int E = 4 * R;
+  uint4 cur_p[R], nxt_p[R];
+  auto fetch = [&](uint4 (&bp)[R], int base) {
+#pragma unroll
+    for (int r = 0; r < R; ++r) {
+      int v = base + r * BLK + (int)threadIdx.x;
+      if (v < nvec) bp[r] = vseg[v];
+      else bp[r] = uint4{ENTRY_PAD32, ENTRY_PAD32, ENTRY_PAD32, ENTRY_PAD32};
+    }
+  };
+  auto pick = [&](int e) {
+    const uint4& q = cur_p[e >> 2];
+    return (e & 3) == 0 ? q.x : (e & 3) == 1 ? q.y : (e & 3) == 2 ? q.z : q.w;
+  };
+  fetch(cur_p, 0);
+  for (int base = 0; base < nvec; base += chunk) {
+    if (base + chunk < nvec) fetch(nxt_p, base + chunk);
+    uint32_t slot[E];
+    unsigned long long first[E];
+#pragma unroll
+    for (int e = 0; e < E; ++e) {
+      slot[e] = (pick(e) >> sshift) & lmask;
+      first[e] = cells[slot[e]];
+    }
+    uint32_t pend = 0, moved = 0;
+#pragma unroll
+    for (int e = 0; e < E; ++e) {
+      uint32_t en = pick(e);
+      if (en == ENTRY_PAD32) continue;
+      if ((uint32_t)(first[e] >> 32) == en) {
+        atomicAdd((unsigned int*)&cells[slot[e]], 1u);
+      } else {
+        pend |= 1u << e;
+        if (first[e] != EMPTY_SLOT) {
+          slot[e] = (slot[e] + 1) & lmask;
+          moved |= 1u << e;
+        }
+      }
+    }
+    if (pend != 0) {
+      drain(
+          pend,
+          [&](int e) {
+            uint32_t v = 0;
+#pragma unroll
+            for (int j = 0; j < E; ++j) {
+              if (j == e) v = pick(j);
+            }
+            return v;
+          },
+          [&](int e) {
+            uint32_t v = 0;
+#pragma unroll
+            for (int j = 0; j < E; ++j) {
+              if (j == e) v = slot[j];
+            }
+            return v;
+          },
+          [&](int e) { return ((moved >> e) & 1u) != 0; });
+    }
+#pragma unroll
+    for (int r = 0; r < R; ++r) cur_p[r] = nxt_p[r];
+  }
+  __syncthreads();
+
+  for (int s = threadIdx.x; s < region; s += BLK) {
+    unsigned long long c = cells[s];
+    if (c != EMPTY_SLOT) {
+      if (!hash_add(tkeys, tvals, mask, region_bits,
+                    compact_classic((uint32_t)b, (uint32_t)(c >> 32), nbits,
+                                    wbase),
+                    c & 0xFFFFFFFFULL)) {
         atomicOr(error_flag, 1);
       }
     }
@@ -3208,6 +3632,10 @@
   const char* s = std::getenv("BYTEWAX_ENTRIES");
   return s != nullptr && s[0] == 'c';
 }
+static bool entries_hashed_env() {
+  const char* s = std::getenv("BYTEWAX_ENTRIES");
+  return s != nullptr && s[0] == 'h';
+}
 
 static bool staged2_shape(int64_t nseg, int* threads, int* u, size_t* lds) {
   int env_u = 0, env_threads = 0;
@@ -3234,19 +3662,31 @@
 
 struct CountEntries {
   bool hashed = false;
+  int dbits = 0;
   int64_t W = 0;
   uint32_t qoff = 0;
   uint32_t dm = 0;
   int sh1 = 0, sh2 = 0;
+  bool compact() const { return dbits > 0; }
+  int fmt() const {
+    return compact() ? ENTRY_FMT_COMPACT
+                     : hashed ? ENTRY_FMT_HASHED : ENTRY_FMT_CLASSIC;
+  }
   int64_t agg_w() const {
     return hashed ? W + (int64_t)qoff : ENTRY_W_CLASSIC;
   }
 };
+
+static int compact_dbits(int64_t nseg) {
+  int s = 0;
+  while (((int64_t)1 << s) < nseg) ++s;
+  return s - 1;
+}
 
 static CountEntries plan_count_entries(
     bool staged_count, int64_t xf, const void* evp, int64_t nseg,
     int64_t cap, int seg_bits, bool ts_i32, int64_t align_ms,
-    int64_t len_ms, int64_t first_base) {
+    int64_t len_ms, int64_t first_base, bool allow_compact = true) {
   CountEntries ce;
   if (!staged_count || !ts_i32 || entries_classic_env() ||
       !count_staged2_ok(xf, evp, nseg) || !count_agg_compact(cap, seg_bits))
@@ -3270,7 +3710,13 @@
   ce.sh1 = l < 1 ? l : 1;
   ce.sh2 = l > 1 ? l - 1 : 0;
   int64_t q0 = (int64_t)((num - w * len_ms + ((__int128)1 << 31)) / len_ms);
-  ce.qoff = q0 > (1 << 18) ? (uint32_t)(q0 - (1 << 18)) : 0u;
+  int64_t back = (int64_t)1 << 18;
+  if (allow_compact && !entries_hashed_env() && nseg >= 128 &&
+      (nseg & (nseg - 1)) == 0 && (cap & ~(int64_t)(SCC_GRAN - 1)) > 0) {
+    ce.dbits = compact_dbits(nseg);
+    back = (int64_t)1 << (ce.dbits - 1);
+  }
+  ce.qoff = q0 > back ? (uint32_t)(q0 - back) : 0u;
   return ce;
 }
 
@@ -3341,6 +3787,22 @@
     if constexpr (sizeof(TSV) == 4) {
       if (ce.hashed) {
         w32 = make_win32(ce, ts_base, align_ms, len_ms);
+        if (ce.compact()) {
+          TORCH_CHECK(nseg == ((int64_t)2 << ce.dbits) && nseg <= 512,
+                      "compact entries planned for another segment count");
+          int64_t gs = (n + 8191) / 8192;
+          unsigned cap_gs = env_blocks > 0 ? (unsigned)env_blocks : cus;
+          if (gs > (int64_t)cap_gs) gs = cap_gs;
+          if (gs < 1) gs = 1;
+          hipLaunchKernelGGL(
+              (k_radix_scatter_compact<16, 512>), dim3((unsigned)gs),
+              dim3(512), compact_lds_bytes(nseg, 8192), stream, keys, ts, n,
+              align_ms, len_ms, ts_base, ce.dbits,
+              cap & ~(int64_t)(SCC_GRAN - 1), gcur, (uint32_t*)evp, ovc, ovp,
+              ov_cap, max_ts, err, win_m2, win_maxfast, w32);
+          HIP_CHECK(hipGetLastError());
+          return;
+        }
         go((k_radix_scatter_staged2<TSV, 16, 512, true>), 512, 16, cus, lds,
            w32);
         return;
@@ -3379,9 +3841,34 @@
     hipStream_t stream, const uint64_t* evp, const int* gcur, int64_t cap,
     uint64_t* tkeys, unsigned long long* tvals, uint64_t mask,
     int region_bits, int seg_bits, int64_t nseg, int* err,
-    int64_t entry_w) {
+    int64_t entry_w, int entry_fmt) {
   const bool hashed = entry_w != ENTRY_W_CLASSIC;
   const uint32_t wlo = hashed ? (uint32_t)(uint64_t)entry_w : 0u;
+  TORCH_CHECK(hashed == (entry_fmt != ENTRY_FMT_CLASSIC),
+              "entry format and entry base disagree");
+  if (entry_fmt == ENTRY_FMT_COMPACT) {
+    TORCH_CHECK(count_agg_compact(cap, seg_bits) && nseg >= 128 &&
+                    (nseg & (nseg - 1)) == 0,
+                "compact entries need the compact-cell aggregation and a "
+                "power-of-two segment count of at least 128");
+    auto go = [&](auto kern, int threads) {
+      hipLaunchKernelGGL(
+          kern, dim3((unsigned)nseg), dim3((unsigned)threads),
+          (size_t)8 << seg_bits, stream, (const uint32_t*)evp, gcur,
+          cap & ~(int64_t)(SCC_GRAN - 1), tkeys, tvals, mask, region_bits,
+          seg_bits, err, wlo, compact_dbits(nseg));
+      HIP_CHECK(hipGetLastError());
+    };
+    int r = 2;
+    if (const char* e = std::getenv("BYTEWAX_AGG_R")) r = atoi(e);
+    if (seg_bits >= 12) {
+      if (r == 1) go((k_radix_agg_compact<1024, 1>), 1024);
+      else go((k_radix_agg_compact<1024, 2>), 1024);
+    } else {
+      go((k_radix_agg_compact<256, 2>), 256);
+    }
+    return;
+  }
   if (count_agg_compact(cap, seg_bits)) {
     auto go = [&](auto kern, int threads) {
       hipLaunchKernelGGL(
@@ -3409,6 +3896,14 @@
 }
 
 static dim3 overflow_agg_grid() { return dim3(device_cu_count()); }
+
+static unsigned long long* spill_total_ptr(
+    const c10::optional<torch::Tensor>& t) {
+  if (!t.has_value()) return nullptr;
+  check_dev(*t, torch::kInt64, "spill_total");
+  TORCH_CHECK(t->numel() >= 1, "spill_total must hold one int64");
+  return (unsigned long long*)t->data_ptr<int64_t>();
+}
 
 static void radix_window_insert_impl(
     torch::Tensor keys,
@@ -3432,7 +3927,9 @@
     int64_t off_ms,
     std::vector<int64_t> seg_counts,
     std::vector<int64_t> seg_bases,
-    const LateSink* late) {
+    const LateSink* late,
+    c10::optional<torch::Tensor> spill_total = c10::nullopt,
+    bool allow_compact = true) {
   if (off_ms <= 0) off_ms = len_ms;
   TORCH_CHECK(off_ms <= len_ms, "window offset must be <= length");
   check_dev(keys, torch::kInt32, "keys");
@@ -3542,7 +4039,7 @@
   const CountEntries ce = plan_count_entries(
       kind == SCAT_STAGED && mode == AGG_COUNT && late == nullptr, xf,
       ev_packed.data_ptr<int64_t>(), nseg, cap, seg_bits, seg32 || ts32,
-      align_ms, len_ms, segs[0].base);
+      align_ms, len_ms, segs[0].base, allow_compact);
   unsigned scat_threads = 256;
   auto scat = [&](auto kern, auto tsptr, const Seg& sg, unsigned gx,
                   size_t lds, auto... extra) {
@@ -3660,7 +4157,7 @@
         (uint64_t*)tkeys.data_ptr<int64_t>(),
         (unsigned long long*)tvals.data_ptr<int64_t>(), mask,
         (int)region_bits, seg_bits, nseg, error_flag.data_ptr<int32_t>(),
-        ce.agg_w());
+        ce.agg_w(), ce.fmt());
   } else {
     agg(k_radix_agg<AGG_SUM>);
   }
@@ -3673,7 +4170,8 @@
         ov_cursor.data_ptr<int32_t>(), ov_packed.numel(),
         (uint64_t*)tkeys.data_ptr<int64_t>(),
         (unsigned long long*)tvals.data_ptr<int64_t>(), mask,
-        (int)region_bits, error_flag.data_ptr<int32_t>());
+        (int)region_bits, error_flag.data_ptr<int32_t>(),
+        spill_total_ptr(spill_total));
   };
   if (mode == AGG_COUNT) ov(k_overflow_agg<AGG_COUNT>);
   else ov(k_overflow_agg<AGG_SUM>);
@@ -3700,12 +4198,14 @@
     int64_t region_bits,
     int64_t off_ms = 0,
     std::vector<int64_t> seg_counts = {},
-    std::vector<int64_t> seg_bases = {}) {
+    std::vector<int64_t> seg_bases = {},
+    c10::optional<torch::Tensor> spill_total = c10::nullopt,
+    bool compact = true) {
   radix_window_insert_impl(
       keys, ts, vals, tkeys, tvals, max_ts, error_flag, gcursors, ev_packed,
       ev_vals, ov_cursor, ov_packed, ov_vals, align_ms, len_ms, mode, ts_base,
       region_bits, off_ms, std::move(seg_counts), std::move(seg_bases),
-      nullptr);
+      nullptr, std::move(spill_total), compact);
 }
 
 void radix_window_insert_late(
@@ -3741,7 +4241,7 @@
       region_bits, off_ms, {}, {}, &sink);
 }
 
-int64_t radix_scatter_only(
+pybind11::object radix_scatter_only(
     torch::Tensor keys,
     torch::Tensor ts,
     c10::optional<torch::Tensor> vals,
@@ -3761,7 +4261,12 @@
     int64_t region_bits,
     int64_t off_ms,
     std::vector<int64_t> seg_counts,
-    std::vector<int64_t> seg_bases) {
+    std::vector<int64_t> seg_bases,
+    bool compact = false) {
+  auto result = [&](const CountEntries& ce) -> pybind11::object {
+    if (!compact) return pybind11::int_(ce.agg_w());
+    return pybind11::make_tuple(ce.agg_w(), ce.fmt());
+  };
   if (off_ms <= 0) off_ms = len_ms;
   TORCH_CHECK(off_ms <= len_ms, "window offset must be <= length");
   check_dev(keys, torch::kInt32, "keys");
@@ -3834,7 +4339,7 @@
       gcursors.data_ptr<int32_t>(), 0, (size_t)nseg * sizeof(int), stream));
   HIP_CHECK(hipMemsetAsync(
       ov_cursor.data_ptr<int32_t>(), 0, sizeof(int), stream));
-  if (n == 0) return ENTRY_W_CLASSIC;
+  if (n == 0) return result(CountEntries{});
 
   struct Seg {
     int64_t off, n, base;
@@ -3849,11 +4354,11 @@
   } else {
     segs.push_back({0, n, ts_base});
   }
-  if (segs.empty()) return ENTRY_W_CLASSIC;
+  if (segs.empty()) return result(CountEntries{});
   const CountEntries ce = plan_count_entries(
       kind == SCAT_STAGED && mode == AGG_COUNT, xf,
       ev_packed.data_ptr<int64_t>(), nseg, cap, seg_bits, seg32 || ts32,
-      align_ms, len_ms, segs[0].base);
+      align_ms, len_ms, segs[0].base, compact);
   unsigned scat_threads = 256;
   auto scat = [&](auto kern, auto tsptr, const Seg& sg, unsigned gx,
                   size_t lds, auto... extra) {
@@ -3912,7 +4417,7 @@
     if (seg32 || ts32) scat_any(ts.data_ptr<int32_t>(), sg);
     else scat_any(ts.data_ptr<int64_t>(), sg);
   }
-  return ce.agg_w();
+  return result(ce);
 }
 
 void radix_agg_only(
@@ -3927,7 +4432,13 @@
     torch::Tensor ov_vals,
     int64_t mode,
     int64_t region_bits,
-    int64_t entry_w = ENTRY_W_CLASSIC) {
+    int64_t entry_w = ENTRY_W_CLASSIC,
+    int64_t entry_fmt = -1,
+    c10::optional<torch::Tensor> spill_total = c10::nullopt) {
+  if (mode != AGG_COUNT) entry_w = ENTRY_W_CLASSIC;
+  if (entry_fmt < 0 || mode != AGG_COUNT)
+    entry_fmt =
+        entry_w != ENTRY_W_CLASSIC ? ENTRY_FMT_HASHED : ENTRY_FMT_CLASSIC;
   int64_t nslots = tkeys.numel();
   int64_t nb = nslots >> region_bits;
   auto stream = at::hip::getCurrentHIPStream();
@@ -3985,7 +4496,7 @@
         (uint64_t*)tkeys.data_ptr<int64_t>(),
         (unsigned long long*)tvals.data_ptr<int64_t>(), mask,
         (int)region_bits, seg_bits, nseg, error_flag.data_ptr<int32_t>(),
-        mode == AGG_COUNT ? entry_w : ENTRY_W_CLASSIC);
+        entry_w, (int)entry_fmt);
   } else {
     agg(k_radix_agg<AGG_SUM>);
   }
@@ -3997,7 +4508,8 @@
         ov_cursor.data_ptr<int32_t>(), ov_packed.numel(),
         (uint64_t*)tkeys.data_ptr<int64_t>(),
         (unsigned long long*)tvals.data_ptr<int64_t>(), mask,
-        (int)region_bits, error_flag.data_ptr<int32_t>());
+        (int)region_bits, error_flag.data_ptr<int32_t>(),
+        spill_total_ptr(spill_total));
   };
   if (mode == AGG_COUNT) ov(k_overflow_agg<AGG_COUNT>);
   else ov(k_overflow_agg<AGG_SUM>);
@@ -5702,14 +6214,15 @@
             (uint64_t*)cur_k.data_ptr<int64_t>(),
             (unsigned long long*)cur_v.data_ptr<int64_t>(), mask,
             (int)region_bits, seg_bits, nseg,
-            error_flag.data_ptr<int32_t>(), ce.agg_w());
+            error_flag.data_ptr<int32_t>(), ce.agg_w(), ce.fmt());
         hipLaunchKernelGGL(
             k_overflow_agg<AGG_COUNT>, overflow_agg_grid(), block, 0, stream,
             (const uint64_t*)ovp.data_ptr<int64_t>(),
             (const int64_t*)nullptr, ovc.data_ptr<int32_t>(), ovp.numel(),
             (uint64_t*)cur_k.data_ptr<int64_t>(),
             (unsigned long long*)cur_v.data_ptr<int64_t>(), mask,
-            (int)region_bits, error_flag.data_ptr<int32_t>());
+            (int)region_bits, error_flag.data_ptr<int32_t>(),
+            (unsigned long long*)nullptr);
         HIP_CHECK(hipEventRecord(ev_ag[par], stream));
       } else if (use_radix) {
         radix_window_insert(
@@ -6181,7 +6694,18 @@
         "scatter (COUNT mode)");
   m.def("radix_scatter_only", &radix_scatter_only,
         "Scatter stage of the radix insert on the current stream; returns "
-        "the entry base for radix_agg_only");
+        "the entry base for radix_agg_only, or with compact=True the pair "
+        "(entry base, entry format)",
+        pybind11::arg("keys"), pybind11::arg("ts"), pybind11::arg("vals"),
+        pybind11::arg("max_ts"), pybind11::arg("error_flag"),
+        pybind11::arg("gcursors"), pybind11::arg("ev_packed"),
+        pybind11::arg("ev_vals"), pybind11::arg("ov_cursor"),
+        pybind11::arg("ov_packed"), pybind11::arg("ov_vals"),
+        pybind11::arg("nslots"), pybind11::arg("align_ms"),
+        pybind11::arg("len_ms"), pybind11::arg("mode"),
+        pybind11::arg("ts_base"), pybind11::arg("region_bits"),
+        pybind11::arg("off_ms"), pybind11::arg("seg_counts"),
+        pybind11::arg("seg_bases"), pybind11::arg("compact") = false);
   m.def("radix_agg_only", &radix_agg_only,
         "Aggregation stage of the radix insert on the current stream",
         pybind11::arg("tkeys"), pybind11::arg("tvals"),
@@ -6190,7 +6714,9 @@
         pybind11::arg("ov_cursor"), pybind11::arg("ov_packed"),
         pybind11::arg("ov_vals"), pybind11::arg("mode"),
         pybind11::arg("region_bits"),
-        pybind11::arg("entry_w") = (int64_t)ENTRY_W_CLASSIC);
+        pybind11::arg("entry_w") = (int64_t)ENTRY_W_CLASSIC,
+        pybind11::arg("entry_fmt") = (int64_t)-1,
+        pybind11::arg("spill_total") = pybind11::none());
   m.def("window_agg_insert_late", &window_agg_insert_late,
         "Single-pass window insert that diverts events below the late "
         "cutoff to a late buffer");
@@ -6204,7 +6730,19 @@
         "Radix stats insert that diverts events below the late cutoff "
         "to a late buffer");
   m.def("radix_window_insert", &radix_window_insert,
-        "Radix-partitioned LDS-staged keyed window aggregation");
+        "Radix-partitioned LDS-staged keyed window aggregation",
+        pybind11::arg("keys"), pybind11::arg("ts"), pybind11::arg("vals"),
+        pybind11::arg("tkeys"), pybind11::arg("tvals"),
+        pybind11::arg("max_ts"), pybind11::arg("error_flag"),
+        pybind11::arg("gcursors"), pybind11::arg("ev_packed"),
+        pybind11::arg("ev_vals"), pybind11::arg("ov_cursor"),
+        pybind11::arg("ov_packed"), pybind11::arg("ov_vals"),
+        pybind11::arg("align_ms"), pybind11::arg("len_ms"),
+        pybind11::arg("mode"), pybind11::arg("ts_base"),
+        pybind11::arg("region_bits"), pybind11::arg("off_ms"),
+        pybind11::arg("seg_counts"), pybind11::arg("seg_bases"),
+        pybind11::arg("spill_total") = pybind11::none(),
+        pybind11::arg("compact") = true);
   m.def("close_migrate", &close_migrate,
         "Window close with reclamation: emit closed cells and migrate "
         "live cells into a fresh table");
diff --git a/bytewax_amd/gpu/__init__.py b/bytewax_amd/gpu/__init__.py
--- a/bytewax_amd/gpu/__init__.py
+++ b/bytewax_amd/gpu/__init__.py
@@ -1,4 +1,5 @@
 
+import logging
 from dataclasses import dataclass
 from datetime import datetime, timezone
 from typing import Any, Dict, Optional, Tuple
@@ -10,6 +11,8 @@
 
 AGG_COUNT = 0
 AGG_SUM = 1
+SPILL_DEMOTE_SHARE = 64
+ENTRY_W_CLASSIC = -(1 << 63)
 
 _INT64_MAX = (1 << 63) - 1
 
@@ -421,6 +424,13 @@
                 1, dtype=torch.int32, device=device
             )
             self._alloc_rx(max(max_batch, 1))
+            self.spill_total = torch.zeros(
+                1, dtype=torch.int64, device=device
+            )
+            self.compact_ok = True
+            self._spill_seen = 0
+            self._ins_since_close = 0
+            self._spill_pin = None
         if self.cpu:
             self._table: Dict[Tuple[int, int], int] = {}
             return
@@ -581,7 +591,10 @@
                 self.off_ms,
                 [],
                 [],
-            )
+                self.spill_total,
+                self.compact_ok,
+            )
+            self._ins_since_close += len(batch)
         else:
             self.k.window_agg_insert(
                 batch.keys,
@@ -677,6 +690,7 @@
         self._pipe_parity = 0
         self._ev_sc = [torch.cuda.Event(), torch.cuda.Event()]
         self._ev_w = [None, None]
+        self._ev_fmt = [None, None]
         self._ev_ag = [torch.cuda.Event(), torch.cuda.Event()]
         self._ag_recorded = [False, False]
         if not hasattr(self, "rx_packed2"):
@@ -740,7 +754,9 @@
             ts.record_stream(self._sc_stream)
             if vals is not None:
                 vals.record_stream(self._sc_stream)
-            self._ev_w[par] = self.k.radix_scatter_only(
+            self._ins_since_close += n
+            compact = self.compact_ok
+            said = self.k.radix_scatter_only(
                 keys,
                 ts,
                 vals,
@@ -756,7 +772,11 @@
                 self.off_ms,
                 list(seg_counts),
                 [int(b) for b in seg_bases],
-            )
+                compact,
+            )
+            if not compact:
+                said = (said, 0 if said == ENTRY_W_CLASSIC else 1)
+            self._ev_w[par], self._ev_fmt[par] = said
             self._ev_sc[par].record(self._sc_stream)
         cur.wait_event(self._ev_sc[par])
         self.k.radix_agg_only(
@@ -767,6 +787,8 @@
             self.mode,
             self.region_bits,
             self._ev_w[par],
+            self._ev_fmt[par],
+            self.spill_total,
         )
         self._ev_ag[par].record(cur)
         self._ag_recorded[par] = True
@@ -803,7 +825,10 @@
             self.off_ms,
             lz.seg_counts,
             lz.seg_bases,
-        )
+            self.spill_total,
+            self.compact_ok,
+        )
+        self._ins_since_close += n
         if lz.max_ts is not None and lz.max_ts > self.max_ts_host:
             self.max_ts_host = lz.max_ts
 
@@ -850,6 +875,8 @@
         _check_error_flag(
             int(self.error_flag.item()), "keyed window state table"
         )
+        if self.radix:
+            self._note_spill(int(self.spill_total.item()))
         if n == 0:
             return None
         return RecordBatch(
@@ -857,6 +884,25 @@
             self.out_wins[:n].to(torch.int64) * self.off_ms + self.align_ms,
             self.out_vals[:n].clone(),
         )
+
+    def _note_spill(self, total: int) -> None:
+        spilled = total - self._spill_seen
+        inserted = self._ins_since_close
+        self._spill_seen = total
+        self._ins_since_close = 0
+        if (
+            self.compact_ok
+            and inserted > 0
+            and spilled * SPILL_DEMOTE_SHARE > inserted
+        ):
+            self.compact_ok = False
+            logging.getLogger(__name__).warning(
+                "keyed window state: %d of %d events since the last close "
+                "went through the overflow spill; keeping 8-byte hashed "
+                "scatter entries from here on",
+                spilled,
+                inserted,
+            )
 
     def _extract_range(self, win_lo: int, win_hi: int) -> Optional[RecordBatch]:
         if self.cpu:
@@ -952,6 +998,14 @@
             )
         self._outn_pin[0:1].copy_(self.out_n, non_blocking=True)
         self._outn_pin[1:2].copy_(self.error_flag, non_blocking=True)
+        if self.radix:
+            if self._spill_pin is None:
+                self._spill_pin = torch.zeros(
+                    1,
+                    dtype=torch.int64,
+                    pin_memory=torch.cuda.is_available(),
+                )
+            self._spill_pin.copy_(self.spill_total, non_blocking=True)
         self._close_ev = torch.cuda.Event()
         self._close_ev.record()
         self._close_pending = True
@@ -967,6 +1021,8 @@
             self._carry_cpu = None
             return out
         self._close_ev.synchronize()
+        if self.radix:
+            self._note_spill(int(self._spill_pin[0].item()))
         n = int(self._outn_pin[0].item())
         _check_error_flag(
             int(self._outn_pin[1].item()), "keyed window state table"
```

New measurement: 134.2 billion events/s, median of 6. 9.4% higher.
